# fenghuayumo/DIVSHOT

Hardware: AMD Instinct MI355X
Metric: train views/sec (fwd+bwd raster) at 1M splats 1920x1080 (higher is better)
Workload: dtype f32; 1 GPU; C3: 1000000 splats, 1920x1080, SH degree 3, 8 views per iteration sharded over 1 GPU(s) (BASELINE config C4), 8 view(s) per GPU per step as 1 multi-view pass(es) of 8 view(s) (dvs_raster_forward_views / dvs_raster_backward_*); absgrad=True, mode=batch, stagger=False, groups=1, views_per_group=8, early_gather=False, a9_chunks=1, async_forward=True, hip_graph=False, fwd_variant=quadrant, grad_mode=0, tile_bounds=canonical, shN_layout=tiled[N/64][45][64]

## Files before the change

### divshot_amd/_lib.py

```python
import ctypes as C
import os

_HERE = os.path.dirname(os.path.abspath(__file__))
LIB_PATH = os.environ.get("DVS_RASTER_LIB") or os.path.join(_HERE, "lib", "libdvsraster.so")


class DvsError(RuntimeError):
    pass


if not os.path.exists(LIB_PATH):
    raise ImportError(
        f"{LIB_PATH} is missing: build it with `make -C divshot_amd/csrc` (or __graft_entry__.build()). "
        "divshot_amd has no CPU fallback.")

lib = C.CDLL(LIB_PATH, mode=C.RTLD_GLOBAL)


class Splats(C.Structure):
    _fields_ = [("pos", C.c_void_p), ("sh0", C.c_void_p), ("shN", C.c_void_p), ("opacity", C.c_void_p),
                ("scale", C.c_void_p), ("rot", C.c_void_p), ("n", C.c_int32), ("_pad", C.c_int32)]


class Camera(C.Structure):
    _fields_ = [("view", C.c_float * 16), ("proj", C.c_float * 16), ("tan_fovx", C.c_float), ("tan_fovy", C.c_float),
                ("focal_x", C.c_float), ("focal_y", C.c_float), ("campos", C.c_float * 3), ("width", C.c_int32),
                ("height", C.c_int32), ("bg", C.c_float * 3)]


class Opts(C.Structure):
    _fields_ = [("sh_degree", C.c_int32), ("antialias", C.c_int32), ("absgrad", C.c_int32), ("accumulate", C.c_int32),
                ("shn_layout", C.c_int32), ("grad_mode", C.c_int32), ("tile_bounds", C.c_int32), ("_reserved", C.c_int32 * 1)]


class FwdState(C.Structure):
    _fields_ = [("radii", C.c_void_p), ("splat2d", C.c_void_p), ("depth", C.c_void_p), ("flags", C.c_void_p), ("tiles_touched", C.c_void_p), ("sorted_tile", C.c_void_p),
                ("sorted_splat", C.c_void_p), ("ranges", C.c_void_p), ("final_T", C.c_void_p), ("n_contrib", C.c_void_p),
                ("num_rendered", C.c_uint64), ("n", C.c_int32), ("width", C.c_int32), ("height", C.c_int32),
                ("tiles_x", C.c_int32), ("tiles_y", C.c_int32), ("_pad", C.c_int32)]


class SplatGrads(C.Structure):
    _fields_ = [("pos", C.c_void_p), ("sh0", C.c_void_p), ("shN", C.c_void_p), ("opacity", C.c_void_p),
                ("scale", C.c_void_p), ("rot", C.c_void_p), ("absgrad2d", C.c_void_p), ("mean2d", C.c_void_p), ("dcolor", C.c_void_p)]


class DensifyParams(C.Structure):
    _fields_ = [("grad_threshold", C.c_float), ("scale_threshold", C.c_float), ("min_opacity", C.c_float), ("max_world_scale", C.c_float),
                ("max_screen_radius", C.c_int32), ("cap_max", C.c_int32), ("seed", C.c_uint32), ("shn_layout", C.c_int32), ("revised_opacity", C.c_int32)]


class AdamGroup(C.Structure):
    _fields_ = [("param", C.c_void_p), ("grad", C.c_void_p), ("m", C.c_void_p), ("v", C.c_void_p), ("count", C.c_uint64),
                ("lr", C.c_float), ("width", C.c_int32), ("layout", C.c_int32), ("active_chunks", C.c_int32)]


class McmcSets(C.Structure):
    _fields_ = [("param", C.c_void_p * 6), ("m", C.c_void_p * 6), ("v", C.c_void_p * 6)]


class SceneSpec(C.Structure):
    _fields_ = [("n", C.c_int32), ("width", C.c_int32), ("height", C.c_int32), ("sh_degree", C.c_int32),
                ("n_cams", C.c_int32), ("seed", C.c_uint64), ("fov_x_deg", C.c_float), ("scale_log_offset", C.c_float)]


_PROTOS = {
    "dvs_create": (C.c_void_p, [C.c_int, C.c_size_t, C.c_int, C.c_int]),
    "dvs_create_views": (C.c_void_p, [C.c_int, C.c_size_t, C.c_int, C.c_int, C.c_int]),
    "dvs_destroy": (None, [C.c_void_p]),
    "dvs_raster_forward_views": (C.c_int, [C.c_void_p, C.c_void_p, C.POINTER(Splats), C.POINTER(Camera), C.c_int, C.POINTER(Opts), C.c_void_p]),
    "dvs_raster_forward_cancel_prepared": (C.c_int, [C.c_void_p]),
    "dvs_raster_forward_views_prepare": (C.c_int, [C.c_void_p, C.c_void_p, C.POINTER(Splats), C.POINTER(Camera), C.c_int, C.POINTER(Opts), C.c_int64, C.c_int64]),
    "dvs_raster_backward_views": (C.c_int, [C.c_void_p, C.c_void_p, C.POINTER(Splats), C.POINTER(Camera), C.c_int, C.POINTER(Opts),
                                            C.c_void_p, C.POINTER(SplatGrads)]),
    "dvs_get_view_state": (C.c_int, [C.c_void_p, C.c_int, C.POINTER(FwdState)]),
    "dvs_raster_forward": (C.c_int, [C.c_void_p, C.c_void_p, C.POINTER(Splats), C.POINTER(Camera), C.POINTER(Opts),
                                     C.c_void_p, C.POINTER(FwdState), C.POINTER(C.c_uint64)]),
    "dvs_raster_backward": (C.c_int, [C.c_void_p, C.c_void_p, C.POINTER(Splats), C.POINTER(Camera), C.POINTER(Opts),
                                      C.c_void_p, C.POINTER(SplatGrads)]),
    "dvs_raster_backward_composite": (C.c_int, [C.c_void_p, C.c_void_p, C.c_void_p, C.POINTER(Opts), C.c_void_p]),
    "dvs_raster_backward_project": (C.c_int, [C.c_void_p, C.c_void_p, C.POINTER(Splats), C.c_void_p, C.POINTER(Opts),
                                              C.POINTER(SplatGrads)]),
    "dvs_raster_backward_project_chunk": (C.c_int, [C.c_void_p, C.c_void_p, C.POINTER(Splats), C.c_void_p, C.POINTER(Opts),
                                                    C.POINTER(SplatGrads), C.c_int64, C.c_int64]),
    "dvs_raster_backward_dcolor": (C.c_int, [C.c_void_p, C.c_void_p, C.c_void_p]),
    "dvs_sh_grad_combine": (C.c_int, [C.c_void_p, C.c_void_p, C.c_int, C.c_void_p, C.c_int, C.c_int, C.c_void_p, C.c_void_p, C.c_void_p,
                                      C.c_void_p, C.c_int, C.c_int]),
    "dvs_shn_relayout": (C.c_int, [C.c_void_p, C.c_void_p, C.c_int, C.c_void_p, C.c_void_p, C.c_int]),
    "dvs_sort_pairs_u32": (C.c_int, [C.c_void_p, C.c_void_p, C.c_void_p, C.c_void_p, C.c_uint64, C.c_int, C.c_int]),
    "dvs_export_sorted_keys": (C.c_int, [C.c_void_p, C.c_void_p, C.c_void_p]),
    "dvs_get_bwd_intermediates": (C.c_int, [C.c_void_p, C.POINTER(C.c_void_p), C.POINTER(C.c_int)]),
    "dvs_keep_bwd_intermediates": (C.c_int, [C.c_void_p, C.c_int]),
    "dvs_set_async": (C.c_int, [C.c_void_p, C.c_int]),
    "dvs_get_num_rendered": (C.c_int, [C.c_void_p, C.c_void_p, C.POINTER(C.c_uint64)]),
    "dvs_get_sort_rank_mode": (C.c_int, [C.c_void_p]),
    "dvs_debug_sort_depth_keys": (C.c_int, [C.c_void_p, C.c_void_p, C.c_void_p, C.c_uint64, C.c_void_p, C.POINTER(C.c_uint32), C.POINTER(C.c_uint32)]),
    "dvs_set_export_sorted_tiles": (C.c_int, [C.c_void_p, C.c_int]),
    "dvs_get_arena_info": (C.c_int, [C.c_void_p, C.POINTER(C.c_uint64), C.POINTER(C.c_uint64), C.POINTER(C.c_uint64), C.POINTER(C.c_uint64)]),
    "dvs_set_backward_variant": (C.c_int, [C.c_void_p, C.c_int]),
    "dvs_debug_record_decisions": (C.c_int, [C.c_void_p, C.c_void_p, C.c_uint64]),
    "dvs_set_forward_variant": (C.c_int, [C.c_void_p, C.c_int]),
    "dvs_set_live_lists": (C.c_int, [C.c_void_p, C.c_int]),
    "dvs_enable_stage_timing": (C.c_int, [C.c_void_p, C.c_int]),
    "dvs_enable_kernel_probe": (C.c_int, [C.c_void_p, C.c_int]),
    "dvs_read_kernel_probe": (C.c_int, [C.c_void_p, C.POINTER(C.c_float), C.POINTER(C.c_int)]),
    "dvs_get_stage_timing": (C.c_int, [C.c_void_p, C.POINTER(C.POINTER(C.c_char_p)), C.POINTER(C.POINTER(C.c_float))]),
    "dvs_memcpy_d2h": (C.c_int, [C.c_void_p, C.c_void_p, C.c_void_p, C.c_size_t]),
    "dvs_memcpy_h2d": (C.c_int, [C.c_void_p, C.c_void_p, C.c_void_p, C.c_size_t]),
    "dvs_device_malloc": (C.c_void_p, [C.c_void_p, C.c_size_t]),
    "dvs_device_free": (None, [C.c_void_p, C.c_void_p]),
    "dvs_comm_create": (C.c_void_p, [C.c_int, C.c_int, C.c_int, C.c_char_p, C.c_int]),
    "dvs_comm_bootstrap": (C.c_int, [C.c_int, C.c_int, C.c_char_p, C.c_int, C.c_void_p]),
    "dvs_comm_destroy": (None, [C.c_void_p]),
    "dvs_comm_rank": (C.c_int, [C.c_void_p]),
    "dvs_comm_world": (C.c_int, [C.c_void_p]),
    "dvs_comm_backend_ranks": (C.c_int, [C.c_void_p]),
    "dvs_comm_backend_name": (C.c_char_p, [C.c_void_p]),
    "dvs_comm_all_reduce_sum_f32": (C.c_int, [C.c_void_p, C.c_void_p, C.c_void_p, C.c_size_t]),
    "dvs_comm_all_reduce_max_i32": (C.c_int, [C.c_void_p, C.c_void_p, C.c_void_p, C.c_size_t]),
    "dvs_comm_reduce_scatter_sum_f32": (C.c_int, [C.c_void_p, C.c_void_p, C.c_void_p, C.c_void_p, C.c_size_t]),
    "dvs_comm_all_gather_f32": (C.c_int, [C.c_void_p, C.c_void_p, C.c_void_p, C.c_void_p, C.c_size_t]),
    "dvs_comm_broadcast": (C.c_int, [C.c_void_p, C.c_void_p, C.c_void_p, C.c_size_t, C.c_int]),
    "dvs_comm_group_start": (C.c_int, [C.c_void_p]),
    "dvs_comm_group_end": (C.c_int, [C.c_void_p]),
    "dvs_last_error": (C.c_char_p, []),
    "dvs_version": (C.c_char_p, []),
    "dvs_synth_splats": (C.c_int, [C.POINTER(SceneSpec)] + [C.c_void_p] * 6),
    "dvs_synth_camera": (C.c_int, [C.POINTER(SceneSpec), C.c_int, C.POINTER(Camera)]),
    "dvs_synth_target": (C.c_int, [C.POINTER(SceneSpec), C.c_int, C.c_void_p]),
    "dvs_make_camera": (C.c_int, [C.c_void_p, C.c_void_p, C.c_float, C.c_int, C.c_int, C.POINTER(Camera)]),
    "dvs_l1_loss_grad": (C.c_int, [C.c_void_p, C.c_void_p, C.c_void_p, C.c_size_t, C.c_void_p, C.c_void_p]),
    "dvs_l1_loss_grad_w": (C.c_int, [C.c_void_p, C.c_void_p, C.c_void_p, C.c_size_t, C.c_float, C.c_void_p, C.c_void_p]),
    "dvs_l2_loss_grad": (C.c_int, [C.c_void_p, C.c_void_p, C.c_void_p, C.c_size_t, C.c_float, C.c_void_p, C.c_void_p]),
    "dvs_ssim_forward": (C.c_int, [C.c_void_p, C.c_void_p, C.c_void_p, C.c_int, C.c_int, C.c_void_p, C.c_void_p, C.c_void_p, C.c_void_p]),
    "dvs_ssim_backward": (C.c_int, [C.c_void_p, C.c_void_p, C.c_void_p, C.c_int, C.c_int, C.c_void_p, C.c_void_p, C.c_void_p, C.c_float,
                                    C.c_void_p, C.c_int]),
    "dvs_loss_l1_ssim_backward": (C.c_int, [C.c_void_p, C.c_void_p, C.c_void_p, C.c_int, C.c_int, C.c_void_p, C.c_void_p, C.c_void_p, C.c_float,
                                            C.c_void_p, C.c_void_p]),
    "dvs_densify_accumulate": (C.c_int, [C.c_void_p, C.c_int, C.c_void_p, C.c_void_p, C.c_int, C.c_int, C.c_void_p, C.c_void_p, C.c_void_p]),
    "dvs_densify_accumulate_rows": (C.c_int, [C.c_void_p, C.c_int, C.c_int, C.c_void_p, C.c_void_p, C.c_int, C.c_int, C.c_void_p, C.c_void_p, C.c_void_p]),
    "dvs_any_view_radius": (C.c_int, [C.c_void_p, C.c_int, C.c_int, C.c_void_p, C.c_void_p]),
    "dvs_densify_plan": (C.c_int, [C.c_void_p, C.c_int, C.c_void_p, C.c_void_p, C.c_void_p, C.c_void_p, C.c_void_p, C.POINTER(DensifyParams),
                                   C.c_void_p, C.c_void_p, C.c_void_p, C.c_void_p]),
    "dvs_densify_apply": (C.c_int, [C.c_void_p, C.c_int, C.c_void_p, C.c_void_p, C.POINTER(DensifyParams), C.c_int, C.c_void_p, C.c_void_p, C.c_int]),
    "dvs_reset_opacity": (C.c_int, [C.c_void_p, C.c_int, C.c_void_p, C.c_float, C.c_void_p, C.c_void_p]),
    "dvs_adam_step": (C.c_int, [C.c_void_p, C.c_void_p, C.c_void_p, C.c_void_p, C.c_void_p, C.c_size_t, C.c_float, C.c_float,
                                C.c_float, C.c_float, C.c_int]),
    "dvs_mcmc_scratch_bytes": (C.c_size_t, [C.c_int]),
    "dvs_mcmc_init_scratch": (C.c_int, [C.c_void_p, C.c_void_p, C.c_int]),
    "dvs_mcmc_relocate": (C.c_int, [C.c_void_p, C.c_int, C.POINTER(McmcSets), C.c_float, C.c_uint32, C.c_int, C.c_void_p, C.c_int, C.c_void_p]),
    "dvs_mcmc_grow": (C.c_int, [C.c_void_p, C.c_int, C.c_int, C.POINTER(McmcSets), C.c_float, C.c_uint32, C.c_int, C.c_void_p, C.c_int]),
    "dvs_mcmc_add_noise": (C.c_int, [C.c_void_p, C.c_int, C.c_void_p, C.c_void_p, C.c_void_p, C.c_void_p, C.c_float, C.c_uint32]),
    "dvs_mcmc_regularize": (C.c_int, [C.c_void_p, C.c_int, C.c_void_p, C.c_void_p, C.c_void_p, C.c_void_p, C.c_float, C.c_float]),
    "dvs_mcmc_add_noise_range": (C.c_int, [C.c_void_p, C.c_int, C.c_int, C.c_int, C.c_void_p, C.c_void_p, C.c_void_p, C.c_void_p, C.c_float, C.c_uint32]),
    "dvs_mcmc_regularize_range": (C.c_int, [C.c_void_p, C.c_int, C.c_int, C.c_int, C.c_void_p, C.c_void_p, C.c_void_p, C.c_void_p, C.c_float, C.c_float]),
    "dvs_adam_step_groups": (C.c_int, [C.c_void_p, C.POINTER(AdamGroup), C.c_int, C.c_float, C.c_float, C.c_float, C.c_int, C.c_void_p,
                                       C.c_int32]),
}
for _name, (_res, _args) in _PROTOS.items():
    _f = getattr(lib, _name)
    _f.restype = _res
    _f.argtypes = _args


def check(status, what="dvs call"):
    if status != 0:
        raise DvsError(f"{what} failed with status {status}: {lib.dvs_last_error().decode()}")
```

### divshot_amd/csrc/dvs_api.cpp

```cpp
#include <hip/hip_runtime.h>
#include <cstdio>
#include <cstdlib>
#include <cstdint>
#include <cstring>
#include <mutex>
#include <string>
#include <vector>
#include "../../include/dvs_raster.h"
#include "dvs_kernels.h"

static thread_local std::string g_last_error;
static void set_error(const char* what, hipError_t e, const char* file, int line) {
    char buf[512];
    snprintf(buf, sizeof buf, "%s: %s (%s:%d)", what, hipGetErrorString(e), file, line);
    g_last_error = buf;
}
void dvs_set_last_error(const char* msg) { g_last_error = msg ? msg : ""; }
#define HIPCHECK(expr)                                                   \
    do {                                                                 \
        hipError_t _e = (expr);                                          \
        if (_e != hipSuccess) { set_error(#expr, _e, __FILE__, __LINE__); return DVS_ERR_HIP; } \
    } while (0)

namespace {
struct Buf {
    void* p = nullptr;
    size_t bytes = 0;
    int ensure(size_t need) {
        if (need <= bytes) return DVS_OK;
        if (p) { (void)hipFree(p); p = nullptr; bytes = 0; }
        size_t want = need + need / 4;
        hipError_t e = hipMalloc(&p, want);
        if (e != hipSuccess) { e = hipMalloc(&p, need); want = need; }
        if (e != hipSuccess) { set_error("hipMalloc", e, __FILE__, __LINE__); p = nullptr; return DVS_ERR_HIP; }
        bytes = want;
#ifdef DVS_EXPERIMENT
        (void)hipMemset(p, 0, want);
#endif
        return DVS_OK;
    }
    void release() { if (p) (void)hipFree(p); p = nullptr; bytes = 0; }
    template <class T> T* as() const { return (T*)p; }
};

DvsCam to_dev_cam(const dvs_camera& c) {
    DvsCam d;
    memcpy(d.view, c.view, sizeof d.view); memcpy(d.proj, c.proj, sizeof d.proj);
    d.tan_fovx = c.tan_fovx; d.tan_fovy = c.tan_fovy; d.focal_x = c.focal_x; d.focal_y = c.focal_y;
    memcpy(d.campos, c.campos, sizeof d.campos);
    d.width = c.width; d.height = c.height; memcpy(d.bg, c.bg, sizeof d.bg);
    return d;
}
int bits_for(uint32_t max_value) { int b = 0; while (max_value) { ++b; max_value >>= 1; } return b; }
}

struct dvs_ctx {
    int device = 0;
    size_t max_splats = 0;
    int max_w = 0, max_h = 0;
    int max_views = 1;
    int n_views = 1;
    Buf radii, splat2d, depth, flags, tiles_touched, rect, rect_sorted, key[2], ids[2];
    Buf inst_tile[2], inst_splat[2];
    uint32_t* live_splat = nullptr;
    uint32_t* live_pos = nullptr;
    bool live_lists = true;
    Buf tmp_keys, tmp_vals;
    bool export_tiles = false;
    int fe_rank_atomic = 0;
    Buf ranges_canon;
    Buf ranges, final_T, n_contrib;
    size_t fe_zero_bytes = 0;
    uint32_t fe_nbv = 0, fe_nsb = 0;
    Buf fe_state;
    Buf fe_hist;
    int fe_seg_n = -1, fe_seg_V = -1;
    uint32_t fe_seg_rows = 0;
    Buf g_rows;
    Buf dcolor;
    uint64_t* total_dev = nullptr;
    uint64_t* total_host = nullptr;
    uint64_t inst_cap = 0;
    uint64_t inst_grow_events = 0;
    bool async_T = false;
    uint64_t* rec_masks = nullptr; uint64_t rec_cap = 0;
    uint64_t overflow_seen = 0;
    dvs_fwd_state st{};
    bool have_fwd = false;
    bool keep_rows = false;
    bool rows_clean = false;
    bool rows_pending = false;
    int64_t proj_next = 0;
    struct Prep {
        bool valid = false;
        int64_t next = 0;
        int n = 0, V = 0;
        dvs_splats p{};
        dvs_opts opts{};
        dvs_camera cams[DVS_MAX_VIEWS];
    } prep;
    int bwd_variant = DVS_BWD_TR;
    int fwd_variant = DVS_FWD_QUADRANT;
    bool timing = false;
    bool probe = false;
    std::vector<hipEvent_t> probe_ev;
    std::vector<int> probe_kind;
    size_t probe_used = 0;
    std::vector<hipEvent_t> events;
    std::vector<const char*> ev_names;
    size_t ev_used = 0;
    std::vector<const char*> out_names;
    std::vector<float> out_ms;
    std::vector<std::pair<const char*, std::pair<size_t, size_t>>> spans;
};

namespace {
struct StageTimer {
    dvs_ctx* c; hipStream_t st;
    StageTimer(dvs_ctx* c_, hipStream_t s) : c(c_), st(s) {}
    size_t mark() {
        if (!c->timing) return 0;
        if (c->ev_used == c->events.size()) { hipEvent_t e; (void)hipEventCreate(&e); c->events.push_back(e); }
        (void)hipEventRecord(c->events[c->ev_used], st);
        return c->ev_used++;
    }
    void span(const char* name, size_t a, size_t b) { if (c->timing) c->spans.push_back({name, {a, b}}); }
};
void timing_reset(dvs_ctx* c) { c->ev_used = 0; c->spans.clear(); }
hipEvent_t probe_event(dvs_ctx* c, hipStream_t st) {
    if (c->probe_used == c->probe_ev.size()) { hipEvent_t e; (void)hipEventCreate(&e); c->probe_ev.push_back(e); }
    hipEvent_t e = c->probe_ev[c->probe_used++];
    (void)hipEventRecord(e, st);
    return e;
}
void timing_collect(dvs_ctx* c, bool append) {
    if (!c->timing) return;
    if (!append) { c->out_names.clear(); c->out_ms.clear(); }
    for (auto& s : c->spans) {
        float ms = 0.f;
        (void)hipEventSynchronize(c->events[s.second.second]);
        (void)hipEventElapsedTime(&ms, c->events[s.second.first], c->events[s.second.second]);
        c->out_names.push_back(s.first); c->out_ms.push_back(ms);
    }
}

bool fe_no_key16() { static const bool v = [] { const char* e = getenv("DVS_FE_NO_KEY16"); return e && e[0] == '1'; }(); return v; }
bool fe_no_fuse() { static const bool v = [] { const char* e = getenv("DVS_FE_NO_FUSE_A6"); return e && e[0] == '1'; }(); return v; }
uint32_t* ranges_ptr(dvs_ctx* c) { return (uint32_t*)((char*)c->ranges.p + c->fe_zero_bytes); }
uint32_t* fe_kred(dvs_ctx* c) { return (uint32_t*)c->ranges.p; }
unsigned long long* fe_super(dvs_ctx* c) { return (unsigned long long*)((char*)c->ranges.p + (size_t)DVS_FE_KRED_WORDS * 4); }
DvsSeg* fe_seg_all(dvs_ctx* c) { return c->fe_state.as<DvsSeg>(); }
DvsSeg* fe_seg_vis(dvs_ctx* c) { return c->fe_state.as<DvsSeg>() + DVS_MAX_VIEWS; }
DvsSeg* fe_seg_tile(dvs_ctx* c) { return c->fe_state.as<DvsSeg>() + 2 * DVS_MAX_VIEWS; }
uint32_t* fe_superexcl(dvs_ctx* c) { return (uint32_t*)(c->fe_state.as<DvsSeg>() + 3 * DVS_MAX_VIEWS); }
uint32_t* fe_totals(dvs_ctx* c) { return fe_superexcl(c) + (size_t)c->max_views * c->fe_nsb; }
uint32_t* fe_block_sums(dvs_ctx* c) { return fe_totals(c) + (size_t)c->max_views * DVS_FE_MAXBINS; }
int ensure_frontend_arenas(dvs_ctx* c) {
    dvs_fe_block_counts((int)c->max_splats, &c->fe_nbv, &c->fe_nsb);
    c->fe_zero_bytes = (size_t)DVS_FE_KRED_WORDS * 4 + (size_t)c->max_views * c->fe_nsb * 8 * DVS_FE_SUPER_STRIDE;
    c->fe_zero_bytes = (c->fe_zero_bytes + 255) & ~(size_t)255;
    int r;
    const size_t state = 3 * DVS_MAX_VIEWS * sizeof(DvsSeg) + ((size_t)c->max_views * c->fe_nsb + (size_t)c->max_views * DVS_FE_MAXBINS + (size_t)c->max_views * c->fe_nbv) * 4;
    if ((r = c->fe_state.ensure(state)) != DVS_OK) return r;
    if ((r = c->fe_hist.ensure(dvs_fe_hist_words((uint64_t)c->max_splats * c->max_views, c->max_views, DVS_FE_MAXBINS) * 4)) != DVS_OK) return r;
    return DVS_OK;
}

int ensure_splat_arenas(dvs_ctx* c, size_t n) {
    int r;
#define ENS(buf, bytes) if ((r = c->buf.ensure(bytes)) != DVS_OK) return r;
    ENS(radii, n * 4) ENS(splat2d, n * 64) ENS(depth, n * 4)
    ENS(flags, n * 4) ENS(tiles_touched, n * 4) ENS(rect, n * 16) ENS(rect_sorted, n * 16)      ENS(key[0], n * 4) ENS(key[1], n * 4) ENS(ids[0], n * 4) ENS(ids[1], n * 4)
    ENS(g_rows, n * 48)
#undef ENS
    return DVS_OK;
}
int ensure_image_arenas(dvs_ctx* c, int w, int h, int views) {
    const size_t P = (size_t)w * h * views;
    const size_t tiles = (size_t)((w + DVS_TILE - 1) / DVS_TILE) * ((h + DVS_TILE - 1) / DVS_TILE) * views;
    int r;
    if ((r = c->ranges.ensure(c->fe_zero_bytes + tiles * 8)) != DVS_OK) return r;
    if ((r = c->ranges_canon.ensure(tiles * 8)) != DVS_OK) return r;
    if ((r = c->final_T.ensure(P * 4)) != DVS_OK) return r;
    if ((r = c->n_contrib.ensure(P * 4)) != DVS_OK) return r;
    return DVS_OK;
}
int ensure_instance_arenas(dvs_ctx* c, uint64_t T) {
    int r;
    if (c->inst_cap && T > c->inst_cap) ++c->inst_grow_events;
    for (int k = 0; k < 2; ++k) {
        if ((r = c->inst_tile[k].ensure(T * 4)) != DVS_OK) return r;
        if ((r = c->inst_splat[k].ensure(T * 4)) != DVS_OK) return r;
    }
    c->inst_cap = c->inst_tile[0].bytes / 4;
    for (int k = 0; k < 2; ++k) {
        if (c->inst_tile[k].bytes / 4 < c->inst_cap) c->inst_cap = c->inst_tile[k].bytes / 4;
        if (c->inst_splat[k].bytes / 4 < c->inst_cap) c->inst_cap = c->inst_splat[k].bytes / 4;
    }
    if (c->inst_cap >= (1ull << 32)) c->inst_cap = (1ull << 32) - 1;
    if ((r = c->fe_hist.ensure(dvs_fe_hist_words(c->inst_cap, c->max_views, 512) * 4)) != DVS_OK) return r;
    return DVS_OK;
}
}

extern "C" {

const char* dvs_last_error(void) { return g_last_error.c_str(); }
const char* dvs_version(void) { return "divshot_amd raster 0.1 (gfx950)"; }

dvs_ctx* dvs_create_views(int device, size_t max_splats, int max_w, int max_h, int max_views) {
    int count = 0;
    hipError_t e = hipGetDeviceCount(&count);
    if (e != hipSuccess || device < 0 || device >= count) {
        g_last_error = "dvs_create: no such HIP device (the rasterizer has no CPU fallback)";
        return nullptr;
    }
    if (max_views < 1 || max_views > DVS_MAX_VIEWS) { g_last_error = "dvs_create_views: max_views must be in [1, 16]"; return nullptr; }
    if ((e = hipSetDevice(device)) != hipSuccess) { set_error("hipSetDevice", e, __FILE__, __LINE__); return nullptr; }
    dvs_ctx* c = new dvs_ctx();
    c->device = device; c->max_splats = max_splats; c->max_w = max_w; c->max_h = max_h; c->max_views = max_views;
    if (const char* v = getenv("DVS_BWD_VARIANT")) {
        c->bwd_variant = v[0] == '0' ? DVS_BWD_BLOCKS : v[0] == '1' ? DVS_BWD_REDUCE : v[0] == '2' ? DVS_BWD_MM : DVS_BWD_TR;
        if ((c->bwd_variant == DVS_BWD_REDUCE || c->bwd_variant == DVS_BWD_MM) && !dvs_launch_render_bwd) c->bwd_variant = DVS_BWD_TR;
    }
    if (const char* v = getenv("DVS_FWD_VARIANT")) c->fwd_variant = (v[0] == '0' && dvs_launch_render_fwd_blocks) ? DVS_FWD_BLOCKS : DVS_FWD_QUADRANT;
    if (const char* v = getenv("DVS_LIVE_LISTS")) c->live_lists = v[0] != '0';
    if (hipMalloc((void**)&c->total_dev, 32) != hipSuccess || hipHostMalloc((void**)&c->total_host, 32, hipHostMallocDefault) != hipSuccess ||
        hipMemset(c->total_dev, 0, 32) != hipSuccess) {
        g_last_error = "dvs_create: hipMalloc failed";
        delete c;
        return nullptr;
    }
    c->total_host[0] = c->total_host[1] = c->total_host[2] = c->total_host[3] = 0;
    {
        static int probed[64];
        static std::mutex probe_mutex;
        std::lock_guard<std::mutex> probe_lock(probe_mutex);
        const char* mode = getenv("DVS_FE_RANK");
        if (mode && mode[0] == 'b') c->fe_rank_atomic = 0;
        else {
            if (device < 64 && probed[device] == 0) {
                uint32_t bad = 1u;
                uint32_t* word = nullptr;
                if (hipMalloc((void**)&word, 4) == hipSuccess && hipMemset(word, 0, 4) == hipSuccess && dvs_fe_probe_rank_atomic(nullptr, word) == hipSuccess &&
                    hipMemcpy(&bad, word, 4, hipMemcpyDeviceToHost) == hipSuccess)
                    probed[device] = bad == 0u ? 1 : 2;
                if (word) (void)hipFree(word);
            }
            c->fe_rank_atomic = (device < 64 && probed[device] == 1) ? 1 : 0;
        }
    }
    if (const char* v = getenv("DVS_ASYNC")) c->async_T = v[0] == '1';
    if (ensure_frontend_arenas(c) != DVS_OK ||
        ensure_splat_arenas(c, max_splats * (size_t)max_views) != DVS_OK || ensure_image_arenas(c, max_w, max_h, max_views) != DVS_OK ||
        ensure_instance_arenas(c, (uint64_t)max_splats * 4 * (uint64_t)max_views) != DVS_OK) {
        dvs_destroy(c);
        return nullptr;
    }
    return c;
}
dvs_ctx* dvs_create(int device, size_t max_splats, int max_w, int max_h) { return dvs_create_views(device, max_splats, max_w, max_h, 1); }

void dvs_destroy(dvs_ctx* c) {
    if (!c) return;
    (void)hipSetDevice(c->device);
    Buf* all[] = {&c->radii, &c->splat2d, &c->depth, &c->flags, &c->tiles_touched, &c->rect, &c->rect_sorted, &c->key[0], &c->key[1],
                  &c->ids[0], &c->ids[1], &c->inst_tile[0], &c->inst_tile[1], &c->inst_splat[0], &c->inst_splat[1],
                  &c->tmp_keys, &c->tmp_vals, &c->ranges, &c->final_T, &c->n_contrib, &c->g_rows, &c->dcolor, &c->fe_state, &c->fe_hist, &c->ranges_canon};
    for (Buf* b : all) b->release();
    if (c->total_dev) (void)hipFree(c->total_dev);
    if (c->total_host) (void)hipHostFree(c->total_host);
    for (hipEvent_t e : c->events) (void)hipEventDestroy(e);
    for (hipEvent_t e : c->probe_ev) (void)hipEventDestroy(e);
    delete c;
}

static int run_a2(dvs_ctx* c, hipStream_t st, const dvs_splats* p, const dvs_camera* cams, int V, const dvs_opts* opts, int64_t first, int64_t count, bool begin) {
    const int n = p->n, W = cams[0].width, H = cams[0].height;
    const int tiles_x = (W + DVS_TILE - 1) / DVS_TILE, tiles_y = (H + DVS_TILE - 1) / DVS_TILE, tiles = tiles_x * tiles_y;
    const int tight = opts->tile_bounds == DVS_TILES_TIGHT ? 1 : 0;
    const int rect_fmt = tight ? DVS_FE_RECT_TIGHT : (tiles_x <= 255 && tiles_y <= 255) ? DVS_FE_RECT_U8 : DVS_FE_RECT_U16;
    DvsCams dcams;
    for (int v = 0; v < V; ++v) dcams.c[v] = to_dev_cam(cams[v]);
    if (begin) HIPCHECK(hipMemsetAsync(c->ranges.p, 0, c->fe_zero_bytes + (size_t)tiles * V * 8, st));
    HIPCHECK(dvs_launch_preprocess_fwd(st, n, p->pos, p->sh0, p->shN, p->opacity, p->scale, p->rot, dcams, V, opts->sh_degree,
                                       opts->antialias, tiles_x, tiles_y, c->radii.as<int>(), c->splat2d.as<float>(),
                                       c->depth.as<float>(), c->flags.as<uint32_t>(), c->tiles_touched.as<uint32_t>(), c->key[0].as<uint32_t>(),
                                       nullptr, opts->shn_layout, rect_fmt == DVS_FE_RECT_U16 ? c->rect.as<uint32_t>() : nullptr,
                                       rect_fmt == DVS_FE_RECT_TIGHT ? c->rect.as<uint32_t>() : nullptr,
                                       rect_fmt == DVS_FE_RECT_U8 ? c->rect.as<uint32_t>() : nullptr, fe_kred(c), (int)first, (int)count));
    return DVS_OK;
}
static bool prep_matches(const dvs_ctx* c, const dvs_splats* p, const dvs_camera* cams, int V, const dvs_opts* opts) {
    const dvs_ctx::Prep& q = c->prep;
    return q.valid && q.n == p->n && q.V == V && memcmp(&q.p, p, sizeof *p) == 0 && memcmp(&q.opts, opts, sizeof *opts) == 0 &&
           memcmp(q.cams, cams, sizeof(dvs_camera) * (size_t)V) == 0;
}

static int forward_views(dvs_ctx* c, hipStream_t st, const dvs_splats* p, const dvs_camera* cams, int V, const dvs_opts* opts,
                         float* out_rgb, dvs_fwd_state* saved, uint64_t* num_rendered) {
    const dvs_camera* cam = &cams[0];
    const int n = p->n, W = cam->width, H = cam->height;
    const int tiles_x = (W + DVS_TILE - 1) / DVS_TILE, tiles_y = (H + DVS_TILE - 1) / DVS_TILE, tiles = tiles_x * tiles_y;
    const size_t nV = (size_t)n * V;
    DvsCams dcams;
    float bgs[DVS_MAX_VIEWS * 3];
    for (int v = 0; v < V; ++v) { dcams.c[v] = to_dev_cam(cams[v]); for (int k = 0; k < 3; ++k) bgs[3 * v + k] = cams[v].bg[k]; }
    c->have_fwd = false;
    c->rows_pending = false;
    timing_reset(c);
    StageTimer tm(c, st);
    const int tight = opts->tile_bounds == DVS_TILES_TIGHT ? 1 : 0;

    uint64_t T = 0, T_expected = 0;
    const uint64_t* T_dev = nullptr;
    int icur = 0;
    size_t e7 = 0;
    int ranges_encoded = 0;
    bool keys_written = true;
    if (c->async_T) {
        const uint64_t lastT = c->total_host[0], overflow = c->total_host[1];
        if (overflow != c->overflow_seen) {
            c->overflow_seen = overflow;
            HIPCHECK(hipStreamSynchronize(st));
            int r = ensure_instance_arenas(c, lastT + lastT / 2);
            if (r != DVS_OK) return r;
            g_last_error = "dvs_raster_forward (async): an earlier forward on this context produced more tile instances than the instance "
                           "arena held; its outputs are invalid. The arena has been enlarged — repeat that view.";
            return DVS_ERR_CAPACITY;
        }
        if (lastT + lastT / 8 > c->inst_cap) {
            HIPCHECK(hipStreamSynchronize(st));
            int r = ensure_instance_arenas(c, lastT + lastT / 2);
            if (r != DVS_OK) return r;
        }
        T = c->inst_cap;
        T_dev = c->total_dev;
        T_expected = lastT > 0 ? lastT + lastT / 16 + 4096 : 0;
    }
    {
        const int rect_fmt = tight ? DVS_FE_RECT_TIGHT : (tiles_x <= 255 && tiles_y <= 255) ? DVS_FE_RECT_U8 : DVS_FE_RECT_U16;
        const bool prepared = prep_matches(c, p, cams, V, opts) && c->prep.next == (int64_t)n;
        c->prep.valid = false;
        size_t e0 = tm.mark();
        if (!prepared) { int r = run_a2(c, st, p, cams, V, opts, 0, n, true); if (r != DVS_OK) return r; }
        size_t e1 = tm.mark(); tm.span("preprocess_fwd", e0, e1);
        if (n > 0) {
            const uint32_t rows = dvs_depth_sort_rows_per_view(n, V);
            if (c->fe_seg_n != n || c->fe_seg_V != V || c->fe_seg_rows != rows) {
                HIPCHECK(dvs_launch_seg_init(st, n, V, rows, fe_seg_all(c)));
                c->fe_seg_n = n; c->fe_seg_V = V; c->fe_seg_rows = rows;
            }
            HIPCHECK(dvs_launch_depth_sort(st, n, V, c->key[0].as<uint32_t>(), c->ids[0].as<uint32_t>(), c->key[1].as<uint32_t>(), c->ids[1].as<uint32_t>(),
                                           fe_seg_all(c), fe_seg_vis(c), fe_kred(c), c->fe_hist.as<uint32_t>(), fe_totals(c), c->fe_rank_atomic));
        }
        size_t e2 = tm.mark(); tm.span("depth_sort", e1, e2);
        const uint64_t lastT = c->total_host[0];
        const uint64_t t_hint = T_expected ? T_expected : (lastT ? lastT : (uint64_t)nV * 3);
        const uint32_t tile_part = dvs_fe_part_for(t_hint);
        if (n > 0)
            HIPCHECK(dvs_launch_seg_binning(st, n, V, rect_fmt, fe_seg_vis(c), fe_seg_tile(c), c->ids[1].as<uint32_t>(), c->rect.as<uint32_t>(),
                                            c->rect_sorted.as<uint32_t>(), fe_block_sums(c), fe_super(c), fe_superexcl(c), tile_part,
                                            (unsigned long long*)c->total_dev, c->async_T ? c->inst_cap : ~0ull, 0, tiles_x, nullptr, nullptr));
        else
            HIPCHECK(hipMemsetAsync(c->total_dev, 0, 8, st));
        HIPCHECK(hipMemcpyAsync(c->total_host, c->total_dev, 32, hipMemcpyDeviceToHost, st));
        size_t e3 = tm.mark(); tm.span("tile_scan", e2, e3);
        if (!c->async_T) {
            HIPCHECK(hipStreamSynchronize(st));
            T = c->total_host[0];
            if (T >= (1ull << 32)) { g_last_error = "dvs_raster_forward: more than 2^32 tile instances"; return DVS_ERR_CAPACITY; }
            { int r = ensure_instance_arenas(c, T ? T : 1); if (r != DVS_OK) return r; }
        }
        const int key16 = (tiles <= 65536 && !fe_no_key16()) ? 1 : 0;
        size_t e4 = tm.mark();
        if (n > 0)
            HIPCHECK(dvs_launch_seg_binning(st, n, V, rect_fmt, fe_seg_vis(c), fe_seg_tile(c), c->ids[1].as<uint32_t>(), c->rect.as<uint32_t>(),
                                            c->rect_sorted.as<uint32_t>(), fe_block_sums(c), fe_super(c), fe_superexcl(c), tile_part,
                                            (unsigned long long*)c->total_dev, c->inst_cap, 1, tiles_x, c->inst_tile[0].as<uint32_t>(),
                                            c->inst_splat[0].as<uint32_t>(), key16));
        size_t e5 = tm.mark(); tm.span("duplicate", e4, e5);
        const bool fuse_a6 = (c->fwd_variant == DVS_FWD_QUADRANT || V > 1) && !fe_no_fuse();
        const bool write_keys = !(fuse_a6 && c->async_T) || c->export_tiles;
        if (n > 0) {
            const uint64_t cap = c->async_T ? c->inst_cap : T;
            const uint32_t nbtot = (uint32_t)(cap / tile_part) + (uint32_t)V + 2u;
            HIPCHECK(dvs_launch_seg_sort(st, V, c->inst_tile[0].as<uint32_t>(), c->inst_splat[0].as<uint32_t>(), c->inst_tile[1].as<uint32_t>(),
                                         c->inst_splat[1].as<uint32_t>(), fe_seg_tile(c), 0, tiles > 1 ? bits_for((uint32_t)(tiles - 1)) : 1,
                                         c->async_T ? (T_expected ? T_expected : c->inst_cap) : T, tile_part, nbtot, c->fe_hist.as<uint32_t>(), fe_totals(c),
                                         (uint32_t)tiles, &icur, fuse_a6 ? ranges_ptr(c) : nullptr, write_keys ? 1 : 0, key16, c->fe_rank_atomic));
        }
        size_t e6 = tm.mark(); tm.span("tile_sort", e5, e6);
        if (fuse_a6) ranges_encoded = n > 0 ? 1 : 0;
        else HIPCHECK(dvs_launch_tile_ranges(st, T, c->inst_tile[icur].as<uint32_t>(), ranges_ptr(c), tiles * V, T_dev, T_expected, false));
        keys_written = write_keys;
        e7 = tm.mark(); tm.span("tile_ranges", e6, e7);
    }
    if (c->probe) { (void)probe_event(c, st); c->probe_kind.push_back(0); }
    c->live_splat = nullptr; c->live_pos = nullptr;
    uint64_t* rec_masks = nullptr; uint64_t rec_cap = 0;
    if (c->rec_masks && V == 1 && !c->async_T && (c->fwd_variant == DVS_FWD_QUADRANT)) {
        rec_masks = c->rec_masks; rec_cap = c->rec_cap;
        HIPCHECK(hipMemsetAsync(rec_masks, 0, (size_t)(T < rec_cap ? T : rec_cap) * 32, st));
    }
    if (c->fwd_variant == DVS_FWD_QUADRANT || V > 1) {
        if (c->live_lists && c->bwd_variant == DVS_BWD_TR) { c->live_splat = c->inst_splat[icur ^ 1].as<uint32_t>(); c->live_pos = c->inst_tile[icur ^ 1].as<uint32_t>(); }
        HIPCHECK(dvs_launch_render_fwd(st, W, H, tiles_x, tiles_y, V, ranges_ptr(c), c->inst_splat[icur].as<uint32_t>(),
                                       c->splat2d.as<float>(), bgs, out_rgb, c->final_T.as<float>(), c->n_contrib.as<uint32_t>(),
                                       c->live_splat, c->live_pos, rec_masks, rec_cap, ranges_encoded ? c->ranges_canon.as<uint32_t>() : nullptr));
    } else
        HIPCHECK(dvs_launch_render_fwd_blocks(st, W, H, tiles_x, tiles_y, ranges_ptr(c), c->inst_splat[icur].as<uint32_t>(),
                                              c->splat2d.as<float>(), cam->bg, out_rgb,
                                              c->final_T.as<float>(), c->n_contrib.as<uint32_t>()));
    if (c->probe) (void)probe_event(c, st);
    size_t e8 = tm.mark(); tm.span("render_fwd", e7, e8);

    dvs_fwd_state& s = c->st;
    s.radii = c->radii.as<int32_t>(); s.splat2d = c->splat2d.as<float>(); s.depth = c->depth.as<float>();
    s.flags = c->flags.as<uint32_t>();
    s.tiles_touched = c->tiles_touched.as<uint32_t>();
    s.sorted_tile = keys_written ? c->inst_tile[icur].as<uint32_t>() : nullptr; s.sorted_splat = c->inst_splat[icur].as<uint32_t>();
    s.ranges = ranges_encoded ? c->ranges_canon.as<uint32_t>() : ranges_ptr(c); s.final_T = c->final_T.as<float>(); s.n_contrib = c->n_contrib.as<uint32_t>();
    s.num_rendered = c->async_T ? DVS_T_UNKNOWN : T; s.n = n; s.width = W; s.height = H; s.tiles_x = tiles_x; s.tiles_y = tiles_y;
    s._pad = 0;
    c->n_views = V;
    c->have_fwd = true;
    if (saved) *saved = s;
    if (num_rendered) *num_rendered = c->async_T ? DVS_T_UNKNOWN : T;
    if (c->timing) { HIPCHECK(hipStreamSynchronize(st)); timing_collect(c, false); }
    return DVS_OK;
}

static int check_fwd_args(dvs_ctx* c, const dvs_splats* p, const dvs_camera* cams, int V, const dvs_opts* opts, const float* out_rgb) {
    if (!c || !p || !cams || !opts || !out_rgb) { g_last_error = "dvs_raster_forward: null argument"; return DVS_ERR_INVALID; }
    if (V < 1 || V > c->max_views) { g_last_error = "dvs_raster_forward: n_views exceeds the max_views given to dvs_create_views"; return DVS_ERR_CAPACITY; }
    const dvs_camera* cam = &cams[0];
    if (p->n < 0 || cam->width <= 0 || cam->height <= 0 || opts->sh_degree < 0 || opts->sh_degree > 3 ||
        (opts->shn_layout != DVS_SHN_ROWS && opts->shn_layout != DVS_SHN_TILED) ||
        (opts->tile_bounds != DVS_TILES_CANONICAL && opts->tile_bounds != DVS_TILES_TIGHT)) {
        g_last_error = "dvs_raster_forward: bad n / image size / sh_degree / shn_layout / tile_bounds"; return DVS_ERR_INVALID;
    }
    for (int v = 1; v < V; ++v)
        if (cams[v].width != cam->width || cams[v].height != cam->height) { g_last_error = "dvs_raster_forward: the views of a batch must share one image size"; return DVS_ERR_INVALID; }
    if (p->n > 0 && (((uintptr_t)p->pos | (uintptr_t)p->sh0 | (uintptr_t)p->shN | (uintptr_t)p->opacity | (uintptr_t)p->scale | (uintptr_t)p->rot) & 15u)) {
        g_last_error = "dvs_raster_forward: parameter arrays must be 16-byte aligned"; return DVS_ERR_INVALID;
    }
    if ((size_t)p->n > c->max_splats || cam->width > c->max_w || cam->height > c->max_h) {
        g_last_error = "dvs_raster_forward: exceeds the capacity given to dvs_create"; return DVS_ERR_CAPACITY;
    }
    if ((uint64_t)p->n * (uint64_t)V >= (1ull << 31)) { g_last_error = "dvs_raster_forward: n * n_views must stay below 2^31"; return DVS_ERR_CAPACITY; }
    return DVS_OK;
}

int dvs_raster_forward(dvs_ctx* c, void* stream, const dvs_splats* p, const dvs_camera* cam, const dvs_opts* opts,
                       float* out_rgb, dvs_fwd_state* saved, uint64_t* num_rendered) {
    int r = check_fwd_args(c, p, cam, 1, opts, out_rgb);
    if (r != DVS_OK) return r;
    HIPCHECK(hipSetDevice(c->device));
    return forward_views(c, (hipStream_t)stream, p, cam, 1, opts, out_rgb, saved, num_rendered);
}

int dvs_raster_forward_views(dvs_ctx* c, void* stream, const dvs_splats* p, const dvs_camera* cams, int n_views, const dvs_opts* opts,
                             float* out_rgb) {
    int r = check_fwd_args(c, p, cams, n_views, opts, out_rgb);
    if (r != DVS_OK) return r;
    HIPCHECK(hipSetDevice(c->device));
    return forward_views(c, (hipStream_t)stream, p, cams, n_views, opts, out_rgb, nullptr, nullptr);
}

int dvs_raster_forward_cancel_prepared(dvs_ctx* c) {
    if (!c) { g_last_error = "dvs_raster_forward_cancel_prepared: null context"; return DVS_ERR_INVALID; }
    c->prep.valid = false;
    return DVS_OK;
}
int dvs_raster_forward_views_prepare(dvs_ctx* c, void* stream, const dvs_splats* p, const dvs_camera* cams, int n_views, const dvs_opts* opts,
                                     int64_t first, int64_t count) {
    static float dummy_rgb;
    int r = check_fwd_args(c, p, cams, n_views, opts, &dummy_rgb);
    if (r != DVS_OK) return r;
    if (opts->shn_layout != DVS_SHN_TILED) { g_last_error = "dvs_raster_forward_views_prepare: needs the DVS_SHN_TILED layout"; return DVS_ERR_INVALID; }
    const bool begin = first == 0;
    if (!begin && !(prep_matches(c, p, cams, n_views, opts) && c->prep.next == first)) {
        c->prep.valid = false;
        g_last_error = "dvs_raster_forward_views_prepare: chunks must cover [0, n) in ascending order with the same parameters, cameras and options";
        return DVS_ERR_STATE;
    }
    if (count <= 0 || first < 0 || first + count > p->n || (first % 256) != 0) {
        c->prep.valid = false;
        g_last_error = "dvs_raster_forward_views_prepare: bad chunk (each starts at a multiple of 256 and lies inside [0, n))"; return DVS_ERR_INVALID;
    }
    HIPCHECK(hipSetDevice(c->device));
    if (begin) {
        c->have_fwd = false; c->rows_pending = false;
        c->prep.valid = true; c->prep.next = 0; c->prep.n = p->n; c->prep.V = n_views; c->prep.p = *p; c->prep.opts = *opts;
        memcpy(c->prep.cams, cams, sizeof(dvs_camera) * (size_t)n_views);
    }
    if ((r = run_a2(c, (hipStream_t)stream, p, cams, n_views, opts, first, count, begin)) != DVS_OK) { c->prep.valid = false; return r; }
    c->prep.next = first + count;
    return DVS_OK;
}

int dvs_get_view_state(dvs_ctx* c, int view, dvs_fwd_state* out) {
    if (!c || !out) { g_last_error = "dvs_get_view_state: null argument"; return DVS_ERR_INVALID; }
    if (!c->have_fwd || view < 0 || view >= c->n_views) { g_last_error = "dvs_get_view_state: no such view in the last forward"; return DVS_ERR_STATE; }
    dvs_fwd_state s = c->st;
    const size_t on = (size_t)view * s.n, op = (size_t)view * s.width * s.height, ot = (size_t)view * s.tiles_x * s.tiles_y;
    s.radii += on; s.splat2d += on * DVS_S2D_FLOATS; s.depth += on; s.flags += on; s.tiles_touched += on;
    s.ranges += 2 * ot; s.final_T += op; s.n_contrib += op;
    *out = s;
    return DVS_OK;
}

static int bwd_composite(dvs_ctx* c, hipStream_t st, const dvs_camera* cams, const dvs_opts* opts, const float* dL_drgb, StageTimer* tm) {
    const dvs_fwd_state& s = c->st;
    const int V = c->n_views;
    size_t e0 = tm ? tm->mark() : 0;
    if (!c->rows_clean) HIPCHECK(hipMemsetAsync(c->g_rows.p, 0, c->g_rows.bytes, st));
    c->rows_clean = false;
    size_t e1 = tm ? tm->mark() : 0;
    if (tm) tm->span("bwd_zero", e0, e1);
    float bgs[DVS_MAX_VIEWS * 3];
    for (int v = 0; v < V; ++v) for (int k = 0; k < 3; ++k) bgs[3 * v + k] = cams[v].bg[k];
    if (c->probe) { (void)probe_event(c, st); c->probe_kind.push_back(1); }
    if (c->bwd_variant == DVS_BWD_TR)
        HIPCHECK(dvs_launch_render_bwd_tr(st, s.width, s.height, s.tiles_x, s.tiles_y, V, s.ranges, s.sorted_splat, s.splat2d, bgs, s.final_T,
                                          s.n_contrib, dL_drgb, c->g_rows.as<float>(), opts->absgrad, opts->grad_mode, c->live_splat, c->live_pos));
    else if (c->bwd_variant == DVS_BWD_BLOCKS)
        HIPCHECK(dvs_launch_render_bwd_blocks(st, s.width, s.height, s.tiles_x, s.tiles_y, V, s.ranges, s.sorted_splat, s.splat2d,
                                              bgs, s.final_T, s.n_contrib, dL_drgb, c->g_rows.as<float>(), opts->absgrad, opts->grad_mode));
    else {
        if (!dvs_launch_render_bwd) { g_last_error = "dvs_raster_backward: this build does not contain the selected composite-backward variant"; return DVS_ERR_INVALID; }
        HIPCHECK(dvs_launch_render_bwd(st, s.width, s.height, s.tiles_x, s.tiles_y, V, s.ranges, s.sorted_splat, s.splat2d,
                                       bgs, s.final_T, s.n_contrib, dL_drgb, c->g_rows.as<float>(), opts->absgrad, opts->grad_mode,
                                       V > 1 ? DVS_BWD_REDUCE : c->bwd_variant));
    }
    if (c->probe) (void)probe_event(c, st);
    if (tm) { size_t e2 = tm->mark(); tm->span("render_bwd", e1, e2); }
    c->rows_pending = true;
    c->proj_next = 0;
    return DVS_OK;
}
static int bwd_project(dvs_ctx* c, hipStream_t st, const dvs_splats* p, const dvs_camera* cams, const dvs_opts* opts,
                       const dvs_splat_grads* out, StageTimer* tm) {
    const dvs_fwd_state& s = c->st;
    const int V = c->n_views, n = p->n;
    size_t e2 = tm ? tm->mark() : 0;
    if (opts->shn_layout == DVS_SHN_TILED) {
        DvsCams dcams;
        float campos[DVS_MAX_VIEWS * 3];
        for (int v = 0; v < V; ++v) { dcams.c[v] = to_dev_cam(cams[v]); for (int k = 0; k < 3; ++k) campos[3 * v + k] = cams[v].campos[k]; }
        const char* nf = getenv("DVS_A9_NO_FUSE_SH");
        const bool no_fuse = nf && nf[0] == '1';
        const bool fuse = !out->dcolor && out->sh0 && out->shN && !no_fuse;
        float* dcol = out->dcolor;
        if (!dcol && !fuse) { int r = c->dcolor.ensure((size_t)V * n * 3 * sizeof(float)); if (r != DVS_OK) return r; dcol = c->dcolor.as<float>(); }
        HIPCHECK(dvs_launch_preprocess_bwd_views(st, n, V, p->pos, p->shN, p->opacity, p->scale, p->rot, dcams, opts->sh_degree,
                                                 opts->antialias, s.radii, s.flags, c->g_rows.as<float>(), out->pos, out->opacity, out->scale,
                                                 out->rot, opts->absgrad ? out->absgrad2d : nullptr, out->mean2d, dcol, opts->accumulate,
                                                 c->keep_rows ? 0 : 1, opts->grad_mode, 0, -1, fuse ? out->sh0 : nullptr, fuse ? out->shN : nullptr));
        if (!fuse && out->sh0 && out->shN)
            HIPCHECK(dvs_launch_sh_grad_combine(st, n, p->pos, opts->sh_degree, V, campos, dcol, out->sh0, out->shN, opts->accumulate, 1));
    } else {
        for (int v = 0; v < V; ++v) {
            const DvsCam dcam = to_dev_cam(cams[v]);
            const size_t on = (size_t)v * n;
            HIPCHECK(dvs_launch_preprocess_bwd(st, n, p->pos, p->shN, p->opacity, p->scale, p->rot, dcam, opts->sh_degree, opts->antialias,
                                               s.radii + on, s.flags + on, c->g_rows.as<float>() + on * 12, out->pos, out->sh0, out->shN,
                                               out->opacity, out->scale, out->rot, opts->absgrad ? out->absgrad2d : nullptr, out->mean2d,
                                               out->dcolor ? out->dcolor + on * 3 : nullptr, (opts->accumulate || v > 0) ? 1 : 0,
                                               c->keep_rows ? 0 : 1, opts->shn_layout, opts->grad_mode));
        }
    }
    c->rows_clean = !c->keep_rows;
    c->rows_pending = c->keep_rows;
    c->proj_next = 0;
    if (tm) { size_t e3 = tm->mark(); tm->span("preprocess_bwd", e2, e3); }
    return DVS_OK;
}
static int check_bwd_args(dvs_ctx* c, const dvs_splats* p, const dvs_camera* cams, int V, const dvs_opts* opts, const char* who) {
    static thread_local std::string msg;
    if (!c || !cams || !opts) { msg = std::string(who) + ": null argument"; g_last_error = msg.c_str(); return DVS_ERR_INVALID; }
    if (opts->grad_mode != DVS_GRAD_TRUE && opts->grad_mode != DVS_GRAD_LINEAGE) { msg = std::string(who) + ": bad grad_mode"; g_last_error = msg.c_str(); return DVS_ERR_INVALID; }
    if (!c->have_fwd || V != c->n_views || (p && c->st.n != p->n) || c->st.width != cams[0].width || c->st.height != cams[0].height) {
        msg = std::string(who) + ": no matching forward on this context"; g_last_error = msg.c_str(); return DVS_ERR_STATE;
    }
    return DVS_OK;
}
static int check_grads(const dvs_splats* p, const dvs_splat_grads* out, const char* who) {
    static thread_local std::string msg;
    if (!p || !out) { msg = std::string(who) + ": null argument"; g_last_error = msg.c_str(); return DVS_ERR_INVALID; }
    if (p->n > 0 && (!out->pos || !out->opacity || !out->scale || !out->rot || ((!out->sh0 || !out->shN) && !out->dcolor))) {
        msg = std::string(who) + ": null gradient row pointer (sh0/shN may be NULL only when dcolor is given)";
        g_last_error = msg.c_str(); return DVS_ERR_INVALID;
    }
    if (p->n > 0 && (((uintptr_t)out->pos | (uintptr_t)out->sh0 | (uintptr_t)out->shN | (uintptr_t)out->opacity | (uintptr_t)out->scale |
                      (uintptr_t)out->rot | (uintptr_t)out->absgrad2d | (uintptr_t)out->mean2d | (uintptr_t)out->dcolor) & 15u)) {
        msg = std::string(who) + ": gradient arrays must be 16-byte aligned"; g_last_error = msg.c_str(); return DVS_ERR_INVALID;
    }
    return DVS_OK;
}

static int backward_views(dvs_ctx* c, void* stream, const dvs_splats* p, const dvs_camera* cams, int V, const dvs_opts* opts,
                          const float* dL_drgb, const dvs_splat_grads* out, const char* who) {
    int r;
    if (!dL_drgb) { g_last_error = "dvs_raster_backward: null argument"; return DVS_ERR_INVALID; }
    if ((uintptr_t)dL_drgb & 15u) { g_last_error = "dvs_raster_backward: dL_drgb must be 16-byte aligned (the composite backward reads it as 16-byte words)"; return DVS_ERR_INVALID; }
    if ((r = check_grads(p, out, who)) != DVS_OK) return r;
    if ((r = check_bwd_args(c, p, cams, V, opts, who)) != DVS_OK) return r;
    HIPCHECK(hipSetDevice(c->device));
    hipStream_t st = (hipStream_t)stream;
    timing_reset(c);
    StageTimer tm(c, st);
    if ((r = bwd_composite(c, st, cams, opts, dL_drgb, &tm)) != DVS_OK) return r;
    if ((r = bwd_project(c, st, p, cams, opts, out, &tm)) != DVS_OK) return r;
    if (c->timing) { HIPCHECK(hipStreamSynchronize(st)); timing_collect(c, true); }
    return DVS_OK;
}
int dvs_raster_backward(dvs_ctx* c, void* stream, const dvs_splats* p, const dvs_camera* cam, const dvs_opts* opts,
                        const float* dL_drgb, const dvs_splat_grads* out) {
    return backward_views(c, stream, p, cam, 1, opts, dL_drgb, out, "dvs_raster_backward");
}
int dvs_raster_backward_views(dvs_ctx* c, void* stream, const dvs_splats* p, const dvs_camera* cams, int n_views, const dvs_opts* opts,
                              const float* dL_drgb, const dvs_splat_grads* out) {
    return backward_views(c, stream, p, cams, n_views, opts, dL_drgb, out, "dvs_raster_backward_views");
}

int dvs_raster_backward_composite(dvs_ctx* c, void* stream, const dvs_camera* cam, const dvs_opts* opts, const float* dL_drgb) {
    int r;
    if (!dL_drgb) { g_last_error = "dvs_raster_backward_composite: null argument"; return DVS_ERR_INVALID; }
    if ((uintptr_t)dL_drgb & 15u) { g_last_error = "dvs_raster_backward_composite: dL_drgb must be 16-byte aligned (the composite backward reads it as 16-byte words)"; return DVS_ERR_INVALID; }
    if (!c) { g_last_error = "dvs_raster_backward_composite: null argument"; return DVS_ERR_INVALID; }
    if ((r = check_bwd_args(c, nullptr, cam, c->n_views, opts, "dvs_raster_backward_composite")) != DVS_OK) return r;
    HIPCHECK(hipSetDevice(c->device));
    timing_reset(c);
    StageTimer tm(c, (hipStream_t)stream);
    if ((r = bwd_composite(c, (hipStream_t)stream, cam, opts, dL_drgb, &tm)) != DVS_OK) return r;
    if (c->timing) { HIPCHECK(hipStreamSynchronize((hipStream_t)stream)); timing_collect(c, true); }
    return DVS_OK;
}

int dvs_raster_backward_project(dvs_ctx* c, void* stream, const dvs_splats* p, const dvs_camera* cam, const dvs_opts* opts,
                                const dvs_splat_grads* out) {
    int r;
    if ((r = check_grads(p, out, "dvs_raster_backward_project")) != DVS_OK) return r;
    if (!c) { g_last_error = "dvs_raster_backward_project: null argument"; return DVS_ERR_INVALID; }
    if ((r = check_bwd_args(c, p, cam, c->n_views, opts, "dvs_raster_backward_project")) != DVS_OK) return r;
    if (!c->rows_pending) { g_last_error = "dvs_raster_backward_project: no dvs_raster_backward_composite on this context"; return DVS_ERR_STATE; }
    if (c->proj_next != 0) {
        g_last_error = "dvs_raster_backward_project: a dvs_raster_backward_project_chunk sequence is in progress on this context (finish it up to n)";
        return DVS_ERR_STATE;
    }
    HIPCHECK(hipSetDevice(c->device));
    timing_reset(c);
    StageTimer tm(c, (hipStream_t)stream);
    if ((r = bwd_project(c, (hipStream_t)stream, p, cam, opts, out, &tm)) != DVS_OK) return r;
    if (c->timing) { HIPCHECK(hipStreamSynchronize((hipStream_t)stream)); timing_collect(c, true); }
    return DVS_OK;
}

int dvs_raster_backward_project_chunk(dvs_ctx* c, void* stream, const dvs_splats* p, const dvs_camera* cam, const dvs_opts* opts,
                                      const dvs_splat_grads* out, int64_t first, int64_t count) {
    int r;
    if ((r = check_grads(p, out, "dvs_raster_backward_project_chunk")) != DVS_OK) return r;
    if (!c) { g_last_error = "dvs_raster_backward_project_chunk: null argument"; return DVS_ERR_INVALID; }
    if ((r = check_bwd_args(c, p, cam, c->n_views, opts, "dvs_raster_backward_project_chunk")) != DVS_OK) return r;
    if (!c->rows_pending) { g_last_error = "dvs_raster_backward_project_chunk: no dvs_raster_backward_composite pending on this context"; return DVS_ERR_STATE; }
    if (opts->shn_layout != DVS_SHN_TILED || !out->dcolor || out->sh0 || out->shN) {
        g_last_error = "dvs_raster_backward_project_chunk: needs the DVS_SHN_TILED layout and the factorised form (out->dcolor given, sh0 / shN NULL)";
        return DVS_ERR_INVALID;
    }
    if (first != c->proj_next || count <= 0 || first + count > p->n || (first % 256) != 0) {
        g_last_error = "dvs_raster_backward_project_chunk: chunks must cover [0, n) in ascending order, each starting at a multiple of 256";
        return DVS_ERR_INVALID;
    }
    HIPCHECK(hipSetDevice(c->device));
    const dvs_fwd_state& s = c->st;
    const int V = c->n_views, n = p->n;
    DvsCams dcams;
    for (int v = 0; v < V; ++v) dcams.c[v] = to_dev_cam(cam[v]);
    timing_reset(c);
    StageTimer tm(c, (hipStream_t)stream);
    const size_t t0 = tm.mark();
    HIPCHECK(dvs_launch_preprocess_bwd_views((hipStream_t)stream, n, V, p->pos, p->shN, p->opacity, p->scale, p->rot, dcams, opts->sh_degree,
                                             opts->antialias, s.radii, s.flags, c->g_rows.as<float>(), out->pos, out->opacity, out->scale,
                                             out->rot, opts->absgrad ? out->absgrad2d : nullptr, out->mean2d, out->dcolor, opts->accumulate,
                                             c->keep_rows ? 0 : 1, opts->grad_mode, (int)first, (int)count));
    { const size_t t1 = tm.mark(); tm.span("preprocess_bwd", t0, t1); }
    if (c->timing) { HIPCHECK(hipStreamSynchronize((hipStream_t)stream)); timing_collect(c, true); }
    c->proj_next = first + count;
    if (c->proj_next == n) { c->rows_clean = !c->keep_rows; c->rows_pending = c->keep_rows; c->proj_next = 0; }
    return DVS_OK;
}

int dvs_sort_pairs_u32(dvs_ctx* c, void* stream, uint32_t* keys, uint32_t* vals, uint64_t n, int bit_lo, int bit_hi) {
    if (!c || (n > 0 && (!keys || !vals)) || bit_lo < 0 || bit_hi > 32 || bit_lo > bit_hi) { g_last_error = "dvs_sort_pairs_u32: bad argument"; return DVS_ERR_INVALID; }
    HIPCHECK(hipSetDevice(c->device));
    hipStream_t st = (hipStream_t)stream;
    if (n == 0) return DVS_OK;
    int r;
    if ((r = c->tmp_keys.ensure(n * 4)) != DVS_OK) return r;
    if ((r = c->tmp_vals.ensure(n * 4)) != DVS_OK) return r;
    uint32_t* k[2] = {keys, c->tmp_keys.as<uint32_t>()};
    uint32_t* v[2] = {vals, c->tmp_vals.as<uint32_t>()};
    int cur = 0;
    {
        if (n > (1ull << 32) - 4097ull) { g_last_error = "dvs_sort_pairs_u32: n must be at most 2^32 - 4097"; return DVS_ERR_CAPACITY; }
        if ((r = c->fe_hist.ensure(dvs_fe_hist_words(n, 1, 512) * 4)) != DVS_OK) return r;
        const uint32_t part = dvs_fe_part_for(n);
        HIPCHECK(dvs_launch_seg_init(st, (int)n, 1, 0, fe_seg_all(c)));
        c->fe_seg_n = -1;
        HIPCHECK(dvs_launch_seg_sort(st, 1, k[0], v[0], k[1], v[1], fe_seg_all(c), bit_lo, bit_hi - bit_lo, n, part, (uint32_t)(n / part) + 3u,
                                     c->fe_hist.as<uint32_t>(), fe_totals(c), 0u, &cur, nullptr, 1, 0, c->fe_rank_atomic));
    }
    if (cur == 1) {
        HIPCHECK(hipMemcpyAsync(keys, k[1], n * 4, hipMemcpyDeviceToDevice, st));
        HIPCHECK(hipMemcpyAsync(vals, v[1], n * 4, hipMemcpyDeviceToDevice, st));
    }
    return DVS_OK;
}

int dvs_debug_sort_depth_keys(dvs_ctx* c, void* stream, const uint32_t* keys, uint64_t n, uint32_t* sorted_ids, uint32_t* n_sorted, uint32_t* digit_bits) {
    if (!c || !keys || !sorted_ids || !n_sorted || n == 0 || n > c->max_splats * (uint64_t)c->max_views || n >= (1ull << 31)) {
        g_last_error = "dvs_debug_sort_depth_keys: bad argument (n must be in [1, max_splats * max_views])"; return DVS_ERR_INVALID;
    }
    HIPCHECK(hipSetDevice(c->device));
    hipStream_t st = (hipStream_t)stream;
    std::vector<uint32_t> h(n);
    HIPCHECK(hipMemcpyAsync(h.data(), keys, n * 4, hipMemcpyDeviceToHost, st));
    HIPCHECK(hipStreamSynchronize(st));
    uint32_t mn = 0xFFFFFFFFu, mx = 0u; bool any = false;
    for (uint32_t k : h) if (k != 0xFFFFFFFFu) { mn = k < mn ? k : mn; mx = k > mx ? k : mx; any = true; }
    uint32_t slots[64 * 16] = {0};
    if (any) { slots[0] = ~mn; slots[1] = mx; }
    HIPCHECK(hipMemcpyAsync(fe_kred(c), slots, sizeof slots, hipMemcpyHostToDevice, st));
    HIPCHECK(hipMemcpyAsync(c->key[0].p, keys, n * 4, hipMemcpyDeviceToDevice, st));
    const uint32_t rows = dvs_depth_sort_rows_per_view((int)n, 1);
    HIPCHECK(dvs_launch_seg_init(st, (int)n, 1, rows, fe_seg_all(c)));
    c->fe_seg_n = -1;
    HIPCHECK(dvs_launch_depth_sort(st, (int)n, 1, c->key[0].as<uint32_t>(), c->ids[0].as<uint32_t>(), c->key[1].as<uint32_t>(), c->ids[1].as<uint32_t>(),
                                   fe_seg_all(c), fe_seg_vis(c), fe_kred(c), c->fe_hist.as<uint32_t>(), fe_totals(c), c->fe_rank_atomic));
    DvsSeg sv;
    HIPCHECK(hipMemcpyAsync(&sv, fe_seg_vis(c), sizeof sv, hipMemcpyDeviceToHost, st));
    HIPCHECK(hipStreamSynchronize(st));
    *n_sorted = sv.count;
    if (digit_bits) *digit_bits = sv.bits;
    HIPCHECK(hipMemcpyAsync(sorted_ids, c->ids[1].p, (size_t)sv.count * 4, hipMemcpyDeviceToDevice, st));
    HIPCHECK(hipMemsetAsync(fe_kred(c), 0, sizeof slots, st));
    c->have_fwd = false;
    return DVS_OK;
}

int dvs_export_sorted_keys(dvs_ctx* c, void* stream, uint64_t* out_keys) {
    if (!c || !out_keys) { g_last_error = "dvs_export_sorted_keys: null argument"; return DVS_ERR_INVALID; }
    if (!c->have_fwd) { g_last_error = "dvs_export_sorted_keys: no forward state"; return DVS_ERR_STATE; }
    if (c->st.num_rendered == DVS_T_UNKNOWN) { uint64_t t; int r = dvs_get_num_rendered(c, stream, &t); if (r != DVS_OK) return r; }
    if (!c->st.sorted_tile) {
        g_last_error = "dvs_export_sorted_keys: the last forward was asynchronous (dvs_set_async) and did not materialise the sorted tile ids; "
                       "export the keys of a synchronous forward";
        return DVS_ERR_STATE;
    }
    HIPCHECK(hipSetDevice(c->device));
    HIPCHECK(dvs_launch_export_keys((hipStream_t)stream, c->st.num_rendered, c->st.sorted_tile, c->st.sorted_splat, c->st.depth, out_keys));
    return DVS_OK;
}

int dvs_shn_relayout(dvs_ctx* c, void* stream, int n, const float* src, float* dst, int to_tiled) {
    if (!c || n < 0 || (n > 0 && (!src || !dst))) { g_last_error = "dvs_shn_relayout: bad argument"; return DVS_ERR_INVALID; }
    HIPCHECK(hipSetDevice(c->device));
    HIPCHECK(dvs_launch_shn_relayout((hipStream_t)stream, n, src, dst, to_tiled));
    return DVS_OK;
}

int dvs_sh_grad_combine(dvs_ctx* c, void* stream, int n, const float* pos, int sh_degree, int n_views, const float* campos,
                        const float* dcolor, float* g_sh0, float* g_shN, int accumulate, int shn_layout) {
    if (!c || n < 0 || n_views < 0 || sh_degree < 0 || sh_degree > 3 || (n > 0 && n_views > 0 && (!pos || !campos || !dcolor || !g_sh0 || !g_shN))) {
        g_last_error = "dvs_sh_grad_combine: bad argument"; return DVS_ERR_INVALID;
    }
    HIPCHECK(hipSetDevice(c->device));
    HIPCHECK(dvs_launch_sh_grad_combine((hipStream_t)stream, n, pos, sh_degree, n_views, campos, dcolor, g_sh0, g_shN, accumulate, shn_layout));
    return DVS_OK;
}

int dvs_raster_backward_dcolor(dvs_ctx* c, void* stream, float* dcolor) {
    if (!c || !dcolor || ((uintptr_t)dcolor & 15u)) { g_last_error = "dvs_raster_backward_dcolor: bad argument (dcolor: 16-byte aligned device array)"; return DVS_ERR_INVALID; }
    if (!c->rows_pending) { g_last_error = "dvs_raster_backward_dcolor: no dvs_raster_backward_composite pending on this context"; return DVS_ERR_STATE; }
    HIPCHECK(hipSetDevice(c->device));
    const dvs_fwd_state& s = c->st;
    HIPCHECK(dvs_launch_dcolor_from_rows((hipStream_t)stream, (int64_t)c->n_views * s.n, s.radii, s.flags, c->g_rows.as<float>(), dcolor));
    return DVS_OK;
}

int dvs_set_async(dvs_ctx* c, int enable) {
    if (!c) { g_last_error = "dvs_set_async: null context"; return DVS_ERR_INVALID; }
    c->async_T = enable != 0;
    return DVS_OK;
}
int dvs_get_num_rendered(dvs_ctx* c, void* stream, uint64_t* T) {
    if (!c || !T) { g_last_error = "dvs_get_num_rendered: null argument"; return DVS_ERR_INVALID; }
    if (!c->have_fwd) { g_last_error = "dvs_get_num_rendered: no forward state"; return DVS_ERR_STATE; }
    HIPCHECK(hipSetDevice(c->device));
    HIPCHECK(hipStreamSynchronize((hipStream_t)stream));
    *T = c->total_host[0];
    c->st.num_rendered = *T;
    if (c->total_host[1] != c->overflow_seen) {
        c->overflow_seen = c->total_host[1];
        (void)ensure_instance_arenas(c, *T + *T / 2);
        g_last_error = "dvs_get_num_rendered: the last forward produced more tile instances than the instance arena held; its outputs are "
                       "invalid. The arena has been enlarged — repeat that view.";
        return DVS_ERR_CAPACITY;
    }
    return DVS_OK;
}

int dvs_get_sort_rank_mode(dvs_ctx* c) { return c ? c->fe_rank_atomic : -1; }
int dvs_set_export_sorted_tiles(dvs_ctx* c, int enable) {
    if (!c) { g_last_error = "dvs_set_export_sorted_tiles: null context"; return DVS_ERR_INVALID; }
    c->export_tiles = enable != 0;
    return DVS_OK;
}

int dvs_get_arena_info(dvs_ctx* c, uint64_t* cap, uint64_t* grows, uint64_t* last_T, uint64_t* overflows) {
    if (!c) { g_last_error = "dvs_get_arena_info: null context"; return DVS_ERR_INVALID; }
    if (cap) *cap = c->inst_cap;
    if (grows) *grows = c->inst_grow_events;
    if (last_T) *last_T = c->total_host[0];
    if (overflows) *overflows = c->total_host[1];
    return DVS_OK;
}

int dvs_debug_record_decisions(dvs_ctx* c, uint64_t* take_masks, uint64_t capacity_instances) {
    if (!c || (take_masks && (((uintptr_t)take_masks & 7u) || capacity_instances == 0))) { g_last_error = "dvs_debug_record_decisions: bad argument"; return DVS_ERR_INVALID; }
    c->rec_masks = take_masks; c->rec_cap = take_masks ? capacity_instances : 0;
    return DVS_OK;
}

int dvs_set_backward_variant(dvs_ctx* c, int variant) {
    if (!c || variant < DVS_BWD_BLOCKS || variant > DVS_BWD_TR) { g_last_error = "dvs_set_backward_variant: bad argument"; return DVS_ERR_INVALID; }
    if ((variant == DVS_BWD_REDUCE || variant == DVS_BWD_MM) && !dvs_launch_render_bwd) {
        g_last_error = "dvs_set_backward_variant: the 'reduce' and 'mm' kernels are retired — this library contains 'tr' (default) and 'blocks' only "
                       "(an experiment build, tools/xbuild.sh, brings them back)";
        return DVS_ERR_UNSUPPORTED;
    }
    c->bwd_variant = variant;
    return DVS_OK;
}
int dvs_set_live_lists(dvs_ctx* c, int enable) {
    if (!c) { g_last_error = "dvs_set_live_lists: null context"; return DVS_ERR_INVALID; }
    c->live_lists = enable != 0;
    return DVS_OK;
}
int dvs_set_forward_variant(dvs_ctx* c, int variant) {
    if (!c || (variant != DVS_FWD_BLOCKS && variant != DVS_FWD_QUADRANT)) { g_last_error = "dvs_set_forward_variant: bad argument"; return DVS_ERR_INVALID; }
    if (variant == DVS_FWD_BLOCKS && !dvs_launch_render_fwd_blocks) {
        g_last_error = "dvs_set_forward_variant: the per-block forward is retired — this library contains the quadrant forward only (tools/xbuild.sh brings it back)";
        return DVS_ERR_UNSUPPORTED;
    }
    c->fwd_variant = variant;
    return DVS_OK;
}

int dvs_keep_bwd_intermediates(dvs_ctx* c, int keep) { if (!c) return DVS_ERR_INVALID; c->keep_rows = keep != 0; return DVS_OK; }

int dvs_get_bwd_intermediates(dvs_ctx* c, const float** rows, int* row_floats) {
    if (!c) return DVS_ERR_INVALID;
    if (rows) *rows = c->g_rows.as<float>();
    if (row_floats) *row_floats = 12;
    return DVS_OK;
}

int dvs_enable_stage_timing(dvs_ctx* c, int enable) { if (!c) return DVS_ERR_INVALID; c->timing = enable != 0; return DVS_OK; }
int dvs_enable_kernel_probe(dvs_ctx* c, int enable) {
    if (!c) return DVS_ERR_INVALID;
    c->probe = enable != 0;
    c->probe_used = 0; c->probe_kind.clear();
    return DVS_OK;
}
int dvs_read_kernel_probe(dvs_ctx* c, float mean_ms[2], int count[2]) {
    if (!c || !mean_ms || !count) return DVS_ERR_INVALID;
    HIPCHECK(hipSetDevice(c->device));
    double sum[2] = {0, 0};
    count[0] = count[1] = 0;
    for (size_t k = 0; k < c->probe_kind.size() && 2 * k + 1 < c->probe_used; ++k) {
        float ms = 0.f;
        HIPCHECK(hipEventSynchronize(c->probe_ev[2 * k + 1]));
        HIPCHECK(hipEventElapsedTime(&ms, c->probe_ev[2 * k], c->probe_ev[2 * k + 1]));
        sum[c->probe_kind[k]] += ms; count[c->probe_kind[k]]++;
    }
    for (int i = 0; i < 2; ++i) mean_ms[i] = count[i] ? (float)(sum[i] / count[i]) : 0.f;
    c->probe_used = 0; c->probe_kind.clear();
    return DVS_OK;
}
int dvs_get_stage_timing(dvs_ctx* c, const char*** names, const float** ms) {
    if (!c) return 0;
    if (names) *names = c->out_names.data();
    if (ms) *ms = c->out_ms.data();
    return (int)c->out_names.size();
}

int dvs_memcpy_d2h(dvs_ctx* c, void* host_dst, const void* dev_src, size_t bytes) {
    if (!c) return DVS_ERR_INVALID;
    HIPCHECK(hipSetDevice(c->device));
    HIPCHECK(hipDeviceSynchronize());
    HIPCHECK(hipMemcpy(host_dst, dev_src, bytes, hipMemcpyDeviceToHost));
    return DVS_OK;
}
int dvs_memcpy_h2d(dvs_ctx* c, void* dev_dst, const void* host_src, size_t bytes) {
    if (!c) return DVS_ERR_INVALID;
    HIPCHECK(hipSetDevice(c->device));
    HIPCHECK(hipMemcpy(dev_dst, host_src, bytes, hipMemcpyHostToDevice));
    return DVS_OK;
}
void* dvs_device_malloc(dvs_ctx* c, size_t bytes) {
    if (!c) return nullptr;
    void* p = nullptr;
    if (hipSetDevice(c->device) != hipSuccess || hipMalloc(&p, bytes ? bytes : 1) != hipSuccess) return nullptr;
    return p;
}
void dvs_device_free(dvs_ctx* c, void* p) { if (c && p) { (void)hipSetDevice(c->device); (void)hipFree(p); } }

}
```

### divshot_amd/csrc/dvs_kernels.h

```cpp
#pragma once
#include <hip/hip_runtime.h>
#include <stdint.h>
#include "dvs_device.h"

hipError_t dvs_launch_preprocess_fwd(hipStream_t st, int n, const float* pos, const float* sh0, const float* shN,
                                     const float* opacity, const float* scale, const float* rot, const DvsCams& cams, int n_views,
                                     int deg, int antialias, int tiles_x, int tiles_y, int* radii , float* splat2d,
                                     float* depth, uint32_t* flags,
                                     uint32_t* tiles_touched, uint32_t* depth_key, uint32_t* ids, int shn_tiled, uint32_t* rect ,
                                     uint32_t* rect16 ,
                                     uint32_t* rect8 = nullptr ,
                                     uint32_t* kred = nullptr ,
                                     int first = 0, int count = -1 );
hipError_t dvs_launch_preprocess_bwd(hipStream_t st, int n, const float* pos, const float* shN, const float* opacity,
                                     const float* scale, const float* rot, const DvsCam& cam, int deg, int antialias,
                                     const int* radii, const uint32_t* flags, float* grad_rows ,
                                     float* g_pos, float* g_sh0, float* g_shN, float* g_opacity, float* g_scale,
                                     float* g_rot, float* out_absgrad2d , float* out_mean2d ,
                                     float* out_dcolor , int accumulate, int rezero_rows, int shn_tiled, int grad_mode);
hipError_t dvs_launch_preprocess_bwd_views(hipStream_t st, int n, int n_views, const float* pos, const float* shN, const float* opacity,
                                           const float* scale, const float* rot, const DvsCams& cams, int deg, int antialias,
                                           const int* radii, const uint32_t* flags, float* grad_rows, float* g_pos, float* g_opacity,
                                           float* g_scale, float* g_rot, float* out_absgrad2d, float* out_mean2d, float* out_dcolor,
                                           int accumulate, int rezero_rows, int grad_mode, int first = 0, int count = -1 ,
                                           float* g_sh0 = nullptr, float* g_shN = nullptr );
hipError_t dvs_launch_sh_grad_combine(hipStream_t st, int n, const float* pos, int deg, int n_views, const float* campos_host,
                                      const float* dcolor, float* g_sh0, float* g_shN, int accumulate, int shn_tiled);
hipError_t dvs_launch_dcolor_from_rows(hipStream_t st, int64_t total, const int* radii, const uint32_t* flags, const float* rows, float* dcolor);
hipError_t dvs_launch_shn_relayout(hipStream_t st, int n, const float* src, float* dst, int to_tiled);

struct DvsSeg {
    uint32_t base;
    uint32_t count;
    uint32_t pstart;
    uint32_t sub;
    uint32_t bits;
    uint32_t _r0, _r1, _r2;
};
enum { DVS_FE_RECT_U8 = 0 , DVS_FE_RECT_U16 = 1 ,
       DVS_FE_RECT_TIGHT = 2  };
#define DVS_FE_KRED_WORDS (DVS_MAX_VIEWS * 64 * 16)
#define DVS_FE_MAXBINS 2048
#define DVS_FE_SUPER_STRIDE 32
size_t dvs_fe_hist_words(uint64_t max_elems, int n_views, int max_bins);
uint32_t dvs_depth_sort_rows_per_view(int n, int V);
uint32_t dvs_fe_part_for(uint64_t grid_elems);
void dvs_fe_block_counts(int n, uint32_t* nbv, uint32_t* nsb);
hipError_t dvs_launch_seg_init(hipStream_t st, int n, int V, uint32_t rows_per_view, DvsSeg* seg_all);
hipError_t dvs_launch_depth_sort(hipStream_t st, int n, int V, uint32_t* keys0, uint32_t* vals0, uint32_t* keys1, uint32_t* vals1,
                                 DvsSeg* seg_all, DvsSeg* seg_vis, const uint32_t* kred, uint32_t* hist, uint32_t* totals ,
                                 int rank_atomic = 0 );
hipError_t dvs_launch_seg_sort(hipStream_t st, int V, uint32_t* keys0, uint32_t* vals0, uint32_t* keys1, uint32_t* vals1, DvsSeg* seg, int bit_lo, int bits,
                               uint64_t grid_elems, uint32_t part, uint32_t nbtot, uint32_t* hist, uint32_t* totals, uint32_t key_add_per_view,
                               int* result_in, uint32_t* ranges_enc = nullptr ,
                               int write_last_keys = 1, int first_keys16 = 0 , int rank_atomic = 0);
hipError_t dvs_fe_probe_rank_atomic(hipStream_t st, uint32_t* bad_dev);
hipError_t dvs_launch_seg_binning(hipStream_t st, int n, int V, int rect_fmt, const DvsSeg* seg_vis, DvsSeg* seg_tile, const uint32_t* sorted_ids,
                                  const uint32_t* rect, uint32_t* rect_sorted, uint32_t* block_sums, unsigned long long* super, uint32_t* superexcl,
                                  uint32_t tile_part, unsigned long long* total_dev, unsigned long long capacity, int stage, int tiles_x,
                                  uint32_t* inst_tile, uint32_t* inst_splat, int key16 = 0 );

hipError_t dvs_launch_tile_ranges(hipStream_t st, uint64_t T, const uint32_t* sorted_tile, uint32_t* ranges, int tiles,
                                  const uint64_t* T_dev = nullptr, uint64_t T_expected = 0, bool clear = true );
hipError_t dvs_launch_export_keys(hipStream_t st, uint64_t T, const uint32_t* sorted_tile, const uint32_t* sorted_splat,
                                  const float* depth, uint64_t* out_keys);

hipError_t dvs_launch_render_fwd(hipStream_t st, int W, int H, int tiles_x, int tiles_y, int n_views, const uint32_t* ranges ,
                                 const uint32_t* sorted_splat, const float* splat2d, const float* bgs, float* out_color, float* final_T,
                                 uint32_t* n_contrib, uint32_t* live_splat , uint32_t* live_pos ,
                                 uint64_t* take_masks ,
                                 uint64_t take_cap, uint32_t* ranges_out = nullptr );
hipError_t dvs_launch_render_bwd(hipStream_t st, int W, int H, int tiles_x, int tiles_y, int n_views, const uint32_t* ranges,
                                 const uint32_t* sorted_splat, const float* splat2d, const float* bgs, const float* final_T, const uint32_t* n_contrib,
                                 const float* dL_dout, float* grad_rows , int absgrad, int grad_mode,
                                 int variant ) __attribute__((weak));
enum { DVS_BWD_BLOCKS = 0 , DVS_BWD_REDUCE = 1 , DVS_BWD_MM = 2 ,
       DVS_BWD_TR = 3  };
enum { DVS_FWD_BLOCKS = 0 , DVS_FWD_QUADRANT = 1  };

hipError_t dvs_launch_render_bwd_tr(hipStream_t st, int W, int H, int tiles_x, int tiles_y, int n_views, const uint32_t* ranges,
                                    const uint32_t* sorted_splat, const float* splat2d, const float* bgs , const float* final_T,
                                    const uint32_t* n_contrib, const float* dL_dout, float* grad_rows, int absgrad, int grad_mode,
                                    const uint32_t* live_splat ,
                                    const uint32_t* live_pos);

hipError_t dvs_launch_render_fwd_blocks(hipStream_t st, int W, int H, int tiles_x, int tiles_y, const uint32_t* ranges,
                                        const uint32_t* sorted_splat, const float* splat2d, const float bg[3], float* out_color,
                                        float* final_T, uint32_t* n_contrib) __attribute__((weak));
hipError_t dvs_launch_render_bwd_blocks(hipStream_t st, int W, int H, int tiles_x, int tiles_y, int n_views, const uint32_t* ranges,
                                        const uint32_t* sorted_splat, const float* splat2d, const float* bgs , const float* final_T,
                                        const uint32_t* n_contrib, const float* dL_dout, float* grad_rows, int absgrad, int grad_mode);
```

### divshot_amd/csrc/frontend.hip

```cpp
#include <cstdlib>
#include "dvs_device.h"
#include "dvs_kernels.h"

#define FE_BLOCK 256
#define FE_WAVES (FE_BLOCK / 64)
#define FE_MAXBINS 2048
#define FE_REORDER_BITS 9
#define FE_CULLED 0xFFFFFFFFu

__device__ __forceinline__ uint32_t fe_lane() { return __builtin_amdgcn_mbcnt_hi(~0u, __builtin_amdgcn_mbcnt_lo(~0u, 0u)); }

__device__ __forceinline__ uint64_t fe_match(uint32_t d, bool valid, uint32_t b) {
    const uint64_t v0 = __ballot(valid);
    uint32_t lo = (uint32_t)v0, hi = (uint32_t)(v0 >> 32);
    for (uint32_t k = 0; k < b; ++k) {
        const uint32_t m = (uint32_t)(((int32_t)(d << (31u - k))) >> 31);
        const uint64_t bal = __ballot(m != 0u);
        lo = lo & ~((uint32_t)bal ^ m);
        hi = hi & ~((uint32_t)(bal >> 32) ^ m);
    }
    const uint64_t peers = ((uint64_t)hi << 32) | lo;
    return valid ? peers : 0ull;
}

__device__ __forceinline__ uint32_t fe_wave_incl_scan(uint32_t v) {
#define FE_DPP_ADD(ctrl, rmask) v += (uint32_t)__builtin_amdgcn_update_dpp(0, (int)v, ctrl, rmask, 0xF, false)
    FE_DPP_ADD(0x111, 0xF); FE_DPP_ADD(0x112, 0xF); FE_DPP_ADD(0x114, 0xF); FE_DPP_ADD(0x118, 0xF);
    FE_DPP_ADD(0x142, 0xA);
    FE_DPP_ADD(0x143, 0xC);
#undef FE_DPP_ADD
    return v;
}
__device__ __forceinline__ uint32_t fe_wave_sum(uint32_t v) { return (uint32_t)__builtin_amdgcn_readlane((int)fe_wave_incl_scan(v), 63); }

__device__ __forceinline__ uint32_t fe_block_excl_scan(uint32_t v, uint32_t* tmp, uint32_t* total) {
    const uint32_t lane = fe_lane(), wave = threadIdx.x >> 6;
    const uint32_t inc = fe_wave_incl_scan(v);
    if (lane == 63) tmp[wave] = inc;
    __syncthreads();
    uint32_t wbase = 0, tot = 0;
#pragma unroll
    for (int w = 0; w < FE_WAVES; ++w) { const uint32_t t = tmp[w]; if ((uint32_t)w < wave) wbase += t; tot += t; }
    __syncthreads();
    *total = tot;
    return wbase + inc - v;
}


template <int ITEMS>
__global__ void __launch_bounds__(FE_BLOCK)
k_seg_hist(const uint32_t* __restrict__ keys, DvsSeg* __restrict__ seg, int V, int adaptive, int pass, int shift_s, int bits_s, int cull,
           uint32_t* __restrict__ hist, uint32_t nbtot, const uint32_t* __restrict__ kred, int key16 ) {
    __shared__ uint32_t h[FE_MAXBINS];
    constexpr uint32_t PART = FE_BLOCK * ITEMS;
    const uint32_t lane = fe_lane(), wave = threadIdx.x >> 6, tid = threadIdx.x;
    const uint32_t view = blockIdx.x % (uint32_t)V, w = blockIdx.x / (uint32_t)V, gv = gridDim.x / (uint32_t)V;
    const uint32_t s_base = seg[view].base, s_count = seg[view].count, s_pstart = seg[view].pstart;
    uint32_t b = (uint32_t)bits_s, shift = (uint32_t)shift_s, sub = 0u;
    if (adaptive) {
        if (pass == 0) {
            uint32_t mn = ~kred[((size_t)view * 64 + lane) * 16], mx = kred[((size_t)view * 64 + lane) * 16 + 1];
#pragma unroll
            for (int d = 32; d >= 1; d >>= 1) {
                const uint32_t omn = __shfl_xor(mn, d, 64), omx = __shfl_xor(mx, d, 64);
                mn = omn < mn ? omn : mn; mx = omx > mx ? omx : mx;
            }
            sub = mn; b = 1u;
            if (mx >= mn) { const uint32_t range = mx - mn; const uint32_t rb = range ? 32u - (uint32_t)__builtin_clz(range) : 0u; b = (rb + 2u) / 3u; if (b < 1u) b = 1u; }
            else sub = 0u;
            if (w == 0 && tid == 0) { seg[view].sub = sub; seg[view].bits = b; }
        } else { sub = seg[view].sub; b = seg[view].bits; }
        shift = (uint32_t)pass * b;
    }
    const uint32_t nbins = 1u << b, dmask = nbins - 1u;
    const uint32_t nparts = (s_count + PART - 1) / PART;
    for (uint32_t p = w; p < nparts; p += gv) {
        for (uint32_t e = tid; e < nbins; e += FE_BLOCK) h[e] = 0u;
        __syncthreads();
        const uint32_t wb = p * PART + wave * (64 * ITEMS);
        uint32_t kreg[ITEMS];
        const uint32_t* const kin = keys + s_base;
        const uint16_t* const kin16 = reinterpret_cast<const uint16_t*>(keys) + s_base;
        const uint32_t i0 = wb + lane, ilast = s_count - 1u;
        if (key16) {
#pragma unroll
            for (int r = 0; r < ITEMS; ++r) { const uint32_t idx = i0 + (uint32_t)r * 64; kreg[r] = kin16[idx < ilast ? idx : ilast]; }
        } else {
#pragma unroll
            for (int r = 0; r < ITEMS; ++r) { const uint32_t idx = i0 + (uint32_t)r * 64; kreg[r] = kin[idx < ilast ? idx : ilast]; }
        }
#pragma unroll
        for (int r = 0; r < ITEMS; ++r) {
            const bool valid = i0 + (uint32_t)r * 64 <= ilast && !(cull && kreg[r] == FE_CULLED);
            if (valid) atomicAdd(&h[((kreg[r] - sub) >> shift) & dmask], 1u);
        }
        __syncthreads();
        const size_t row = (size_t)s_pstart + p;
        for (uint32_t d = tid; d < nbins; d += FE_BLOCK) hist[(size_t)d * nbtot + row] = h[d];
        __syncthreads();
    }
}

__global__ void __launch_bounds__(FE_BLOCK)
k_seg_rowscan(uint32_t* __restrict__ hist, uint32_t nbtot, const DvsSeg* __restrict__ seg, int V, int adaptive, int bits_s, uint32_t part,
              uint32_t* __restrict__ totals) {
    const uint32_t lane = fe_lane(), wave = threadIdx.x >> 6;
    const uint32_t view = blockIdx.x % (uint32_t)V, d = (blockIdx.x / (uint32_t)V) * FE_WAVES + wave;
    const uint32_t b = adaptive ? seg[view].bits : (uint32_t)bits_s;
    if (d >= (1u << b)) return;
    const uint32_t nparts = (seg[view].count + part - 1) / part;
    uint32_t* row = hist + (size_t)d * nbtot + seg[view].pstart;
    uint32_t carry = 0;
    for (uint32_t c0 = 0; c0 < nparts; c0 += 1024) {
        uint32_t v[16];
#pragma unroll
        for (int k = 0; k < 16; ++k) { const uint32_t i = c0 + (uint32_t)k * 64 + lane; v[k] = i < nparts ? row[i] : 0u; }
#pragma unroll
        for (int k = 0; k < 16; ++k) {
            if (c0 + (uint32_t)k * 64 < nparts) {
                const uint32_t i = c0 + (uint32_t)k * 64 + lane;
                const uint32_t inc = fe_wave_incl_scan(v[k]);
                if (i < nparts) row[i] = carry + inc - v[k];
                carry += (uint32_t)__builtin_amdgcn_readlane((int)inc, 63);
            }
        }
    }
    if (lane == 0) totals[(size_t)view * FE_MAXBINS + d] = carry;
}

template <int ITEMS> struct FeScatterLds {
    static constexpr int PART = FE_BLOCK * ITEMS;
    static constexpr int REORDER_WORDS = 1024 + 512 + 2 * PART;
    static constexpr int WIDE_WORDS = 4096 + 2048 + 2048;
    static constexpr int WORDS = (REORDER_WORDS > WIDE_WORDS ? REORDER_WORDS : WIDE_WORDS) + 8;
};

template <int ITEMS, bool RANK_ATOMIC >
__global__ void __launch_bounds__(FE_BLOCK) __attribute__((amdgpu_waves_per_eu(4)))
k_seg_scatter(const uint32_t* __restrict__ keys_in, const uint32_t* __restrict__ vals_in ,
              uint32_t* __restrict__ keys_out , uint32_t* __restrict__ vals_out,
              const DvsSeg* __restrict__ seg_in, DvsSeg* __restrict__ seg_out ,
              int V, int adaptive, int pass, int shift_s, int bits_s, int cull, uint32_t key_add_per_view,
              const uint32_t* __restrict__ hist, uint32_t nbtot, const uint32_t* __restrict__ totals,
              int key16 ,
              uint32_t* __restrict__ ranges_enc ) {
    constexpr uint32_t PART = FE_BLOCK * ITEMS;
    __shared__ __attribute__((aligned(16))) uint32_t lds[FeScatterLds<ITEMS>::WORDS];
    const uint32_t lane = fe_lane(), wave = threadIdx.x >> 6, tid = threadIdx.x;
    const uint32_t view = blockIdx.x % (uint32_t)V, w = blockIdx.x / (uint32_t)V, gv = gridDim.x / (uint32_t)V;
    const DvsSeg S = seg_in[view];
    const uint32_t b = adaptive ? S.bits : (uint32_t)bits_s;
    const uint32_t shift = adaptive ? (uint32_t)pass * b : (uint32_t)shift_s;
    const uint32_t sub = adaptive ? S.sub : 0u;
    const uint32_t nbins = 1u << b, dmask = nbins - 1u;
    const bool wide = b > FE_REORDER_BITS;
    const uint32_t cstride = wide ? 2048u : 512u;
    uint16_t* const cnt16 = reinterpret_cast<uint16_t*>(lds);
    uint32_t* const gdelta = lds + (wide ? 4096 : 1024);
    uint32_t* const dexl = lds + 6144;
    uint32_t* const stage_k = lds + 1536;
    uint32_t* const stage_v = stage_k + PART;
    uint32_t* const tmp = lds + (FeScatterLds<ITEMS>::WORDS - 8);
    const uint32_t key_add = key_add_per_view * view;
    const uint32_t* const vtot = totals + (size_t)view * FE_MAXBINS;
    const uint32_t* const kin = keys_in + S.base;
    const uint16_t* const kin16 = reinterpret_cast<const uint16_t*>(keys_in) + S.base;
    const uint32_t* const vin = vals_in ? vals_in + S.base : nullptr;
    uint32_t* const kout = keys_out ? keys_out + S.base : nullptr;
    uint32_t* const vout = vals_out + S.base;

    const uint32_t nparts = (S.count + PART - 1) / PART;
    const uint32_t ilast = S.count - 1u;
    uint32_t key[ITEMS], val[ITEMS], rank[ITEMS];
    constexpr bool EARLY = ITEMS <= 8;
    auto request = [&](uint32_t p) {
        const uint32_t i0 = p * PART + wave * (64 * ITEMS) + lane;
        if (key16) {
#pragma unroll
            for (int r = 0; r < ITEMS; ++r) { const uint32_t idx = i0 + (uint32_t)r * 64; key[r] = kin16[idx < ilast ? idx : ilast]; }
        } else {
#pragma unroll
            for (int r = 0; r < ITEMS; ++r) { const uint32_t idx = i0 + (uint32_t)r * 64; key[r] = kin[idx < ilast ? idx : ilast]; }
        }
        if (vin) {
#pragma unroll
            for (int r = 0; r < ITEMS; ++r) { const uint32_t idx = i0 + (uint32_t)r * 64; val[r] = vin[idx < ilast ? idx : ilast]; }
        } else {
#pragma unroll
            for (int r = 0; r < ITEMS; ++r) val[r] = i0 + (uint32_t)r * 64;
        }
    };
    if (EARLY && w < nparts) request(w);

    uint32_t dex0 = 0, dex1 = 0;
    {
        uint32_t s = 0;
        if (!wide) {
            const uint32_t t0 = 2u * tid < nbins ? vtot[2u * tid] : 0u, t1 = 2u * tid + 1u < nbins ? vtot[2u * tid + 1u] : 0u;
            dex1 = t0; s = t0 + t1;
        } else {
#pragma unroll 1
            for (uint32_t k = 0; k < 8; ++k) { const uint32_t d = tid * 8u + k; s += d < nbins ? vtot[d] : 0u; }
        }
        uint32_t tot;
        const uint32_t off = fe_block_excl_scan(s, tmp, &tot);
        if (!wide) { dex0 = off; dex1 += off; }
        else {
            uint32_t run = off;
#pragma unroll 1
            for (uint32_t k = 0; k < 8; ++k) { const uint32_t d = tid * 8u + k; dexl[d] = run; run += d < nbins ? vtot[d] : 0u; }
        }
        if (seg_out && w == 0 && tid == 0) { seg_out[view].base = S.base; seg_out[view].count = tot; seg_out[view].pstart = S.pstart; seg_out[view].sub = S.sub; seg_out[view].bits = S.bits; }
    }
    for (uint32_t p = w; p < nparts; p += gv) {
        const size_t row = (size_t)S.pstart + p;
        __syncthreads();
        for (uint32_t e = tid; e < cstride * 2u; e += FE_BLOCK) lds[e] = 0u;
        uint32_t hp0 = 0, hp1 = 0;
        if (!wide) {
            if (2u * tid < nbins) hp0 = hist[(size_t)(2u * tid) * nbtot + row];
            if (2u * tid + 1u < nbins) hp1 = hist[(size_t)(2u * tid + 1u) * nbtot + row];
        }
        if (!EARLY) request(p);
        __syncthreads();
        const uint32_t i0 = p * PART + wave * (64 * ITEMS) + lane;
        uint32_t vmask = 0u;
#pragma unroll
        for (int r = 0; r < ITEMS; ++r) {
            const bool valid = i0 + (uint32_t)r * 64 <= ilast && !(cull && key[r] == FE_CULLED);
            const uint32_t d = ((key[r] - sub) >> shift) & dmask;
            uint32_t prev = 0;
            if constexpr (RANK_ATOMIC) {
                if (valid) {
                    const uint32_t old = atomicAdd(&lds[wave * (cstride >> 1) + (d >> 1)], (d & 1u) ? 0x10000u : 1u);
                    prev = (d & 1u) ? (old >> 16) : (old & 0xFFFFu);
                    vmask |= 1u << r;
                }
                rank[r] = prev;
            } else {
                const uint64_t peers = fe_match(d, valid, b);
                const uint32_t below = __builtin_amdgcn_mbcnt_hi((uint32_t)(peers >> 32), __builtin_amdgcn_mbcnt_lo((uint32_t)peers, 0u));
                if (valid) {
                    prev = cnt16[wave * cstride + d];
                    if (below == 0) cnt16[wave * cstride + d] = (uint16_t)(prev + (uint32_t)__popcll(peers));
                    vmask |= 1u << r;
                }
                rank[r] = prev + below;
            }
            asm volatile("" : "+v"(rank[r]));
        }
        __syncthreads();
        if (!wide) {
            uint32_t c0[FE_WAVES], c1[FE_WAVES], bc0 = 0, bc1 = 0;
#pragma unroll
            for (int wv = 0; wv < FE_WAVES; ++wv) {
                const uint32_t two = *reinterpret_cast<const uint32_t*>(&cnt16[(uint32_t)wv * 512u + tid * 2u]);
                c0[wv] = two & 0xFFFFu; c1[wv] = two >> 16; bc0 += c0[wv]; bc1 += c1[wv];
            }
            uint32_t nvalid;
            uint32_t run = fe_block_excl_scan(bc0 + bc1, tmp, &nvalid);
            gdelta[tid * 2u] = dex0 + hp0 - run;
            gdelta[tid * 2u + 1u] = dex1 + hp1 - (run + bc0);
            uint32_t run1 = run + bc0;
#pragma unroll
            for (int wv = 0; wv < FE_WAVES; ++wv) {
                *reinterpret_cast<uint32_t*>(&cnt16[(uint32_t)wv * 512u + tid * 2u]) = run | (run1 << 16);
                run += c0[wv]; run1 += c1[wv];
            }
            __syncthreads();
#pragma unroll
            for (int r = 0; r < ITEMS; ++r) {
                if (vmask & (1u << r)) {
                    uint32_t kk = key[r];
                    asm volatile("" : "+v"(kk));
                    const uint32_t pos = cnt16[wave * 512u + (((kk - sub) >> shift) & dmask)] + rank[r];
                    stage_k[pos] = key[r];
                    stage_v[pos] = val[r];
                }
            }
            __syncthreads();
#pragma unroll
            for (int i = 0; i < ITEMS; ++i) {
                const uint32_t slot = (uint32_t)i * FE_BLOCK + tid;
                if (slot < nvalid) {
                    const uint32_t k = stage_k[slot];
                    const uint32_t dst = gdelta[((k - sub) >> shift) & dmask] + slot;
                    if (kout) kout[dst] = k + key_add;
                    vout[dst] = stage_v[slot];
                    if (ranges_enc) {
                        const uint32_t kp = slot > 0 ? stage_k[slot - 1] : ~k, kn = slot + 1 < nvalid ? stage_k[slot + 1] : ~k;
                        uint32_t* const e = ranges_enc + 2 * (size_t)(key_add + k);
                        const uint32_t at = S.base + dst;
                        if (kp != k) atomicMax(e, ~at);
                        if (kn != k) atomicMax(e + 1, at + 1u);
                    }
                }
            }
            if (EARLY && p + gv < nparts) request(p + gv);
        } else {
#pragma unroll 1
            for (uint32_t k = 0; k < 8; ++k) {
                const uint32_t d = tid * 8u + k;
                uint32_t acc = 0;
#pragma unroll
                for (int wv = 0; wv < FE_WAVES; ++wv) { const uint32_t cw = cnt16[(uint32_t)wv * 2048u + d]; cnt16[(uint32_t)wv * 2048u + d] = (uint16_t)acc; acc += cw; }
                gdelta[d] = dexl[d] + (d < nbins ? hist[(size_t)d * nbtot + row] : 0u);
            }
            __syncthreads();
#pragma unroll
            for (int r = 0; r < ITEMS; ++r) {
                if (vmask & (1u << r)) {
                    uint32_t kk = key[r];
                    asm volatile("" : "+v"(kk));
                    const uint32_t d = ((kk - sub) >> shift) & dmask;
                    const uint32_t dst = gdelta[d] + cnt16[wave * 2048u + d] + rank[r];
                    if (kout) kout[dst] = key[r] + key_add;
                    vout[dst] = val[r];
                }
            }
            if (EARLY && p + gv < nparts) request(p + gv);
        }
    }
}

static inline int fe_items_for(uint64_t n_total) {
    static const uint64_t thr = [] { const char* e = getenv("DVS_FE_ITEMS8_BELOW"); return e ? (uint64_t)atoll(e) : 1500000ull; }();
    return n_total <= thr ? 8 : 16;
}

size_t dvs_fe_hist_words(uint64_t max_elems, int n_views, int max_bins) {
    const uint64_t rows = (max_elems + (uint64_t)FE_BLOCK * 8 - 1) / ((uint64_t)FE_BLOCK * 8) + (uint64_t)n_views + 6;
    return (size_t)(rows * (uint64_t)max_bins);
}

struct FeSortLaunch {
    hipStream_t st;
    int V;
    int items;
    uint32_t grid_per_view;
    uint32_t* hist; uint32_t nbtot; uint32_t* totals;
    int rank_atomic;
};

static hipError_t fe_launch_pass(const FeSortLaunch& L, const uint32_t* kin, const uint32_t* vin, uint32_t* kout, uint32_t* vout, DvsSeg* seg_in,
                                 DvsSeg* seg_out, int adaptive, int pass, int shift, int bits, int cull, uint32_t key_add_per_view,
                                 const uint32_t* kred, uint32_t* ranges_enc = nullptr, int key16 = 0) {
    const dim3 grid(L.grid_per_view * (uint32_t)L.V), blk(FE_BLOCK);
    const int maxbins = adaptive ? FE_MAXBINS : (1 << bits);
    const dim3 rgrid((uint32_t)((maxbins + FE_WAVES - 1) / FE_WAVES) * (uint32_t)L.V);
#define FE_PASS(I, A)                                                                                                                          \
    do {                                                                                                                                       \
        hipLaunchKernelGGL(k_seg_hist<I>, grid, blk, 0, L.st, kin, seg_in, L.V, adaptive, pass, shift, bits, cull, L.hist, L.nbtot, kred, key16); \
        hipLaunchKernelGGL(k_seg_rowscan, rgrid, blk, 0, L.st, L.hist, L.nbtot, (const DvsSeg*)seg_in, L.V, adaptive, bits, (uint32_t)(FE_BLOCK * I), L.totals); \
        hipLaunchKernelGGL((k_seg_scatter<I, A>), grid, blk, 0, L.st, kin, vin, kout, vout, (const DvsSeg*)seg_in, seg_out, L.V, adaptive, pass, shift, bits, \
                           cull, key_add_per_view, (const uint32_t*)L.hist, L.nbtot, (const uint32_t*)L.totals, key16, ranges_enc);               \
    } while (0)
    if (L.items == 8) { if (L.rank_atomic) FE_PASS(8, true); else FE_PASS(8, false); }
    else { if (L.rank_atomic) FE_PASS(16, true); else FE_PASS(16, false); }
#undef FE_PASS
    return hipGetLastError();
}

hipError_t dvs_launch_depth_sort(hipStream_t st, int n, int V, uint32_t* keys0, uint32_t* vals0, uint32_t* keys1, uint32_t* vals1,
                                 DvsSeg* seg_all, DvsSeg* seg_vis, const uint32_t* kred, uint32_t* hist, uint32_t* totals, int rank_atomic) {
    if (n <= 0 || V <= 0) return hipSuccess;
    FeSortLaunch L;
    L.st = st; L.V = V; L.items = fe_items_for((uint64_t)n * V); L.rank_atomic = rank_atomic;
    const uint32_t part = (uint32_t)FE_BLOCK * L.items;
    L.grid_per_view = ((uint32_t)n + part - 1) / part;
    L.hist = hist; L.nbtot = L.grid_per_view * (uint32_t)V + 1; L.totals = totals;
    hipError_t e;
    if ((e = fe_launch_pass(L, keys0, nullptr, keys1, vals1, seg_all, seg_vis, 1, 0, 0, 0, 1, 0, kred)) != hipSuccess) return e;
    if ((e = fe_launch_pass(L, keys1, vals1, keys0, vals0, seg_vis, nullptr, 1, 1, 0, 0, 0, 0, nullptr)) != hipSuccess) return e;
    return fe_launch_pass(L, keys0, vals0, nullptr, vals1, seg_vis, nullptr, 1, 2, 0, 0, 0, 0, nullptr);
}
uint32_t dvs_depth_sort_rows_per_view(int n, int V) {
    const uint32_t part = (uint32_t)FE_BLOCK * fe_items_for((uint64_t)n * V);
    return ((uint32_t)n + part - 1) / part;
}

static void fe_split_bits(int bits, int* npass, int widths[4]) {
    int np = (bits + FE_REORDER_BITS - 1) / FE_REORDER_BITS;
    if (np < 1) np = 1;
    if (np > 4) np = 4;
    int left = bits;
    for (int k = 0; k < np; ++k) { const int wdt = (left + (np - k) - 1) / (np - k); widths[k] = wdt > 0 ? wdt : 1; left -= wdt; }
    *npass = np;
}
uint32_t dvs_fe_part_for(uint64_t grid_elems) { return (uint32_t)FE_BLOCK * (uint32_t)fe_items_for(grid_elems); }

hipError_t dvs_launch_seg_sort(hipStream_t st, int V, uint32_t* keys0, uint32_t* vals0, uint32_t* keys1, uint32_t* vals1, DvsSeg* seg, int bit_lo, int bits,
                               uint64_t grid_elems, uint32_t part, uint32_t nbtot, uint32_t* hist, uint32_t* totals, uint32_t key_add_per_view,
                               int* result_in, uint32_t* ranges_enc, int write_last_keys, int first_keys16, int rank_atomic) {
    if (result_in) *result_in = 0;
    if (V <= 0 || bits <= 0) return hipSuccess;
    int npass, widths[4];
    fe_split_bits(bits, &npass, widths);
    FeSortLaunch L;
    L.st = st; L.V = V; L.items = (int)(part / FE_BLOCK); L.rank_atomic = rank_atomic;
    uint64_t per_view = (grid_elems + (uint64_t)V - 1) / (uint64_t)V;
    uint64_t g = (per_view + part - 1) / part + 1;
    if (g > 65535u * 16u) g = 65535u * 16u;
    L.grid_per_view = (uint32_t)(g < 1 ? 1 : g);
    L.hist = hist; L.nbtot = nbtot; L.totals = totals;
    uint32_t* kk[2] = {keys0, keys1};
    uint32_t* vv[2] = {vals0, vals1};
    int c = 0, shift = bit_lo;
    for (int k = 0; k < npass; ++k) {
        const bool last = k == npass - 1;
        hipError_t e = fe_launch_pass(L, kk[c], vv[c], (last && !write_last_keys) ? nullptr : kk[c ^ 1], vv[c ^ 1], seg, nullptr, 0, k, shift, widths[k], 0,
                                      last ? key_add_per_view : 0u, nullptr, last ? ranges_enc : nullptr, (k == 0 && first_keys16) ? 1 : 0);
        if (e != hipSuccess) return e;
        shift += widths[k];
        c ^= 1;
    }
    if (result_in) *result_in = c;
    return hipSuccess;
}

__global__ void __launch_bounds__(FE_BLOCK)
k_fe_probe_rank_atomic(uint32_t* __restrict__ bad, uint32_t seed) {
    __shared__ uint32_t cnt_a[FE_WAVES * 256];
    __shared__ uint16_t cnt_b[FE_WAVES * 512];
    const uint32_t lane = fe_lane(), wave = threadIdx.x >> 6;
    uint32_t errs = 0;
    for (uint32_t pat = 0; pat < 24; ++pat) {
        for (uint32_t e = threadIdx.x; e < FE_WAVES * 256; e += FE_BLOCK) cnt_a[e] = 0u;
        for (uint32_t e = threadIdx.x; e < FE_WAVES * 512; e += FE_BLOCK) cnt_b[e] = 0;
        __syncthreads();
        const uint32_t bits = pat < 8 ? 9u : 1u + (pat - 8u) % 9u;
        for (uint32_t r = 0; r < 16; ++r) {
            uint32_t h = (lane * 0x9E3779B1u) ^ ((blockIdx.x * FE_WAVES + wave) * 0x85EBCA6Bu) ^ ((pat * 16u + r) * 0xC2B2AE35u) ^ seed;
            h ^= h >> 15; h *= 0x2C1B3C6Du; h ^= h >> 12;
            uint32_t d;
            switch (pat) {
                case 0: d = 5u; break;
                case 1: d = 6u + (lane & 1u); break;
                case 2: d = lane >> 1; break;
                case 3: d = lane / 3u; break;
                case 4: d = lane >> 5; break;
                case 5: d = lane & 7u; break;
                case 6: d = (lane & 1u) ? 511u : (h & 3u); break;
                case 7: d = 63u - lane; break;
                default: d = h & ((1u << bits) - 1u); break;
            }
            const bool valid = (h >> 20 & 15u) != 0u || pat < 8;
            uint32_t ra = 0, rb = 0;
            if (valid) {
                const uint32_t old = atomicAdd(&cnt_a[wave * 256u + (d >> 1)], (d & 1u) ? 0x10000u : 1u);
                ra = (d & 1u) ? (old >> 16) : (old & 0xFFFFu);
            }
            const uint64_t peers = fe_match(d, valid, 9u);
            const uint32_t below = __builtin_amdgcn_mbcnt_hi((uint32_t)(peers >> 32), __builtin_amdgcn_mbcnt_lo((uint32_t)peers, 0u));
            if (valid) {
                const uint32_t prev = cnt_b[wave * 512u + d];
                if (below == 0) cnt_b[wave * 512u + d] = (uint16_t)(prev + (uint32_t)__popcll(peers));
                rb = prev + below;
            }
            errs += (valid && ra != rb) ? 1u : 0u;
        }
        __syncthreads();
    }
    if (errs) atomicAdd(bad, errs);
}
hipError_t dvs_fe_probe_rank_atomic(hipStream_t st, uint32_t* bad_dev ) {
    hipLaunchKernelGGL(k_fe_probe_rank_atomic, dim3(512), dim3(FE_BLOCK), 0, st, bad_dev, 0x1234567u);
    hipLaunchKernelGGL(k_fe_probe_rank_atomic, dim3(512), dim3(FE_BLOCK), 0, st, bad_dev, 0x89ABCDEu);
    return hipGetLastError();
}

template <int FMT> struct FeRect;
template <> struct FeRect<DVS_FE_RECT_U8> {
    typedef uint32_t T;
    static __device__ __forceinline__ uint32_t count(T r) { return ((r >> 16) & 0xFFu) * (r >> 24); }
    static __device__ __forceinline__ uint32_t minx(T r) { return r & 0xFFu; }
    static __device__ __forceinline__ uint32_t miny(T r) { return (r >> 8) & 0xFFu; }
    static __device__ __forceinline__ uint32_t width(T r) { return (r >> 16) & 0xFFu; }
    static __device__ __forceinline__ T zero() { return 0u; }
};
template <> struct FeRect<DVS_FE_RECT_U16> {
    typedef uint2 T;
    static __device__ __forceinline__ uint32_t count(T r) { return ((r.x >> 16) - (r.x & 0xFFFFu)) * ((r.y >> 16) - (r.y & 0xFFFFu)); }
    static __device__ __forceinline__ uint32_t minx(T r) { return r.x & 0xFFFFu; }
    static __device__ __forceinline__ uint32_t miny(T r) { return r.y & 0xFFFFu; }
    static __device__ __forceinline__ uint32_t width(T r) { return (r.x >> 16) - (r.x & 0xFFFFu); }
    static __device__ __forceinline__ T zero() { return make_uint2(0u, 0u); }
};
template <> struct FeRect<DVS_FE_RECT_TIGHT> {
    typedef uint4 T;
    static __device__ __forceinline__ uint32_t count(T r) {
        const uint32_t both = r.z & r.w;
        return both == 0xFFFFFFFFu ? ((r.x >> 16) - (r.x & 0xFFFFu)) * ((r.y >> 16) - (r.y & 0xFFFFu)) : (uint32_t)(__popc(r.z) + __popc(r.w));
    }
    static __device__ __forceinline__ uint32_t minx(T r) { return r.x & 0xFFFFu; }
    static __device__ __forceinline__ uint32_t miny(T r) { return r.y & 0xFFFFu; }
    static __device__ __forceinline__ uint32_t width(T r) { return (r.x >> 16) - (r.x & 0xFFFFu); }
    static __device__ __forceinline__ T zero() { return make_uint4(0u, 0u, 0u, 0u); }
};

template <int FMT>
__global__ void __launch_bounds__(FE_BLOCK)
k_seg_blocksum(int n, int V, uint32_t nbv, uint32_t nsb, const DvsSeg* __restrict__ seg_vis, const uint32_t* __restrict__ sorted_ids,
               const typename FeRect<FMT>::T* __restrict__ rect, typename FeRect<FMT>::T* __restrict__ rect_sorted,
               uint32_t* __restrict__ block_sums, unsigned long long* __restrict__ super) {
    __shared__ uint32_t wsum[4][FE_WAVES];
    const uint32_t view = blockIdx.x % (uint32_t)V, blk0 = (blockIdx.x / (uint32_t)V) * 4u;
    const uint32_t nvis = seg_vis[view].count;
    if (blk0 * FE_BLOCK >= nvis) return;
    const size_t o = (size_t)view * n;
    const uint32_t lane = fe_lane(), wave = threadIdx.x >> 6;
    uint32_t id[4];
#pragma unroll
    for (int k = 0; k < 4; ++k) { const uint32_t j = (blk0 + (uint32_t)k) * FE_BLOCK + threadIdx.x; id[k] = j < nvis ? sorted_ids[o + j] : 0u; }
    typename FeRect<FMT>::T r[4];
#pragma unroll
    for (int k = 0; k < 4; ++k) r[k] = rect[o + id[k]];
#pragma unroll
    for (int k = 0; k < 4; ++k) {
        const uint32_t j = (blk0 + (uint32_t)k) * FE_BLOCK + threadIdx.x;
        uint32_t v = 0;
        if (j < nvis) { rect_sorted[o + j] = r[k]; v = FeRect<FMT>::count(r[k]); }
        const uint32_t s = fe_wave_sum(v);
        if (lane == 0) wsum[k][wave] = s;
    }
    __syncthreads();
    if (threadIdx.x < 4) {
        const uint32_t k = threadIdx.x, blk = blk0 + k;
        uint32_t tot = 0;
#pragma unroll
        for (int wv = 0; wv < FE_WAVES; ++wv) tot += wsum[k][wv];
        if (blk < nbv) block_sums[(size_t)view * nbv + blk] = tot;
        const uint32_t t4 = tot + (uint32_t)__shfl_down(tot, 1, 64) + (uint32_t)__shfl_down(tot, 2, 64) + (uint32_t)__shfl_down(tot, 3, 64);
        if (k == 0 && t4) atomicAdd(&super[((size_t)view * nsb + (blk0 >> 8)) * DVS_FE_SUPER_STRIDE], (unsigned long long)t4);
    }
}

__global__ void __launch_bounds__(1024)
k_seg_totals(int V, uint32_t nsb, const unsigned long long* __restrict__ super, uint32_t* __restrict__ superexcl, DvsSeg* __restrict__ seg_tile,
             uint32_t tile_part, unsigned long long* __restrict__ total, unsigned long long capacity) {
    __shared__ unsigned long long vsum[DVS_MAX_VIEWS];
    const uint32_t lane = fe_lane(), wave = threadIdx.x >> 6;
    if (wave < (uint32_t)V) {
        unsigned long long carry = 0ull;
        for (uint32_t c0 = 0; c0 < nsb; c0 += 64) {
            const uint32_t i = c0 + lane;
            const unsigned long long v = i < nsb ? super[((size_t)wave * nsb + i) * DVS_FE_SUPER_STRIDE] : 0ull;
            unsigned long long inc = v;
#pragma unroll
            for (int k = 1; k < 64; k <<= 1) { const unsigned long long o = __shfl_up(inc, k, 64); if (lane >= (uint32_t)k) inc += o; }
            const unsigned long long ex = carry + inc - v;
            if (i < nsb) superexcl[(size_t)wave * nsb + i] = ex > 0xFFFFFFFFull ? 0xFFFFFFFFu : (uint32_t)ex;
            carry += __shfl(inc, 63, 64);
        }
        if (lane == 0) vsum[wave] = carry;
    }
    __syncthreads();
    if (threadIdx.x == 0) {
        unsigned long long start = 0ull;
        uint32_t prow = 0;
        for (int v = 0; v < V; ++v) {
            const unsigned long long end = start + vsum[v];
            const unsigned long long cs = start < capacity ? start : capacity, ce = end < capacity ? end : capacity;
            DvsSeg s;
            s.base = (uint32_t)cs; s.count = (uint32_t)(ce - cs); s.pstart = prow; s.sub = 0u; s.bits = 0u; s._r0 = s._r1 = s._r2 = 0u;
            seg_tile[v] = s;
            prow += (s.count + tile_part - 1) / tile_part;
            start = end;
        }
        total[0] = start;
        if (start > capacity) total[1] += 1ull;
    }
}

__device__ __forceinline__ uint32_t fe_nth_set_bit64(uint32_t lo, uint32_t hi, uint32_t t) {
    uint32_t w = lo, base = 0;
    const uint32_t c = (uint32_t)__popc(lo);
    if (t >= c) { t -= c; w = hi; base = 32u; }
#pragma unroll
    for (uint32_t h = 16u; h >= 1u; h >>= 1) {
        const uint32_t cl = (uint32_t)__popc(w & ((1u << h) - 1u));
        if (t >= cl) { t -= cl; w >>= h; base += h; }
    }
    return base;
}

__device__ __forceinline__ uint32_t fe_wave_incl_max(uint32_t v) {
#define FE_DPP_MAX(ctrl, rmask) { const uint32_t o_ = (uint32_t)__builtin_amdgcn_update_dpp(0, (int)v, ctrl, rmask, 0xF, false); v = v > o_ ? v : o_; }
    FE_DPP_MAX(0x111, 0xF); FE_DPP_MAX(0x112, 0xF); FE_DPP_MAX(0x114, 0xF); FE_DPP_MAX(0x118, 0xF);
    FE_DPP_MAX(0x142, 0xA);
    FE_DPP_MAX(0x143, 0xC);
#undef FE_DPP_MAX
    return v;
}
template <int FMT>
__global__ void __launch_bounds__(FE_BLOCK)
k_seg_duplicate(int n, int V, uint32_t nbv, uint32_t nsb, const DvsSeg* __restrict__ seg_vis, const DvsSeg* __restrict__ seg_tile,
                const uint32_t* __restrict__ sorted_ids, const typename FeRect<FMT>::T* __restrict__ rect_sorted,
                const uint32_t* __restrict__ block_sums, const uint32_t* __restrict__ superexcl, int tiles_x,
                uint32_t* __restrict__ inst_tile, uint32_t* __restrict__ inst_splat, unsigned long long capacity, int key16 ) {
    __shared__ uint32_t tmp[FE_WAVES];
    __shared__ uint32_t s_pre[FE_BLOCK];
    __shared__ uint32_t s_id[FE_BLOCK];
    __shared__ uint32_t s_tile[FE_BLOCK];
    __shared__ uint32_t s_w[FE_BLOCK];
    __shared__ uint32_t s_mark[FE_BLOCK];
    __shared__ uint2 s_mask[FMT == DVS_FE_RECT_TIGHT ? FE_BLOCK : 1];
    const uint32_t view = blockIdx.x % (uint32_t)V, blk0 = (blockIdx.x / (uint32_t)V) * 2u;
    const uint32_t nvis = seg_vis[view].count;
    if (blk0 * FE_BLOCK >= nvis) return;
    const size_t o = (size_t)view * n;
    const uint32_t lane = fe_lane(), w0 = (threadIdx.x >> 6) * 64u;
    uint32_t id[2] = {0u, 0u};
    typename FeRect<FMT>::T r[2] = {FeRect<FMT>::zero(), FeRect<FMT>::zero()};
#pragma unroll
    for (int h = 0; h < 2; ++h) {
        const uint32_t j = (blk0 + (uint32_t)h) * FE_BLOCK + threadIdx.x;
        if (j < nvis) { id[h] = sorted_ids[o + j]; r[h] = rect_sorted[o + j]; }
    }
    const uint32_t sb = blk0 >> 8, nprev = blk0 & 255u;
    const uint32_t part = threadIdx.x < nprev ? block_sums[(size_t)view * nbv + (size_t)sb * 256 + threadIdx.x] : 0u;
    const unsigned long long vbase = (unsigned long long)seg_tile[view].base + superexcl[(size_t)view * nsb + sb];
    uint32_t before, tot;
    (void)fe_block_excl_scan(part, tmp, &before);
#pragma unroll
    for (int h = 0; h < 2; ++h) {
        if ((blk0 + (uint32_t)h) * FE_BLOCK >= nvis) break;
        const uint32_t touched = FeRect<FMT>::count(r[h]);
        const uint32_t pre = fe_block_excl_scan(touched, tmp, &tot);
        s_pre[threadIdx.x] = pre;
        s_id[threadIdx.x] = (uint32_t)o + id[h];
        s_tile[threadIdx.x] = FeRect<FMT>::miny(r[h]) * (uint32_t)tiles_x + FeRect<FMT>::minx(r[h]);
        s_w[threadIdx.x] = FeRect<FMT>::width(r[h]);
        if constexpr (FMT == DVS_FE_RECT_TIGHT) s_mask[threadIdx.x] = make_uint2(r[h].z, r[h].w);
        const unsigned long long gbase = vbase + before;
        const uint32_t k_beg = (uint32_t)__builtin_amdgcn_readfirstlane((int)pre);
        const uint32_t k_end = (uint32_t)__builtin_amdgcn_readlane((int)(pre + touched), 63);
        uint32_t cur1 = 0;
        for (uint32_t k0 = k_beg; k0 < k_end; k0 += 64u) {
            s_mark[w0 + lane] = 0u;
            __builtin_amdgcn_wave_barrier();
            const uint32_t rel = pre - k0;
            if (touched != 0u && rel < 64u) s_mark[w0 + rel] = lane + 1u;
            __builtin_amdgcn_wave_barrier();
            uint32_t m = s_mark[w0 + lane];
            __builtin_amdgcn_wave_barrier();
            m = fe_wave_incl_max(m);
            m = m > cur1 ? m : cur1;
            cur1 = (uint32_t)__builtin_amdgcn_readlane((int)m, 63);
            const uint32_t k = k0 + lane;
            if (k < k_end) {
                const uint32_t src = w0 + m - 1u, w = s_w[src];
                uint32_t t = k - s_pre[src];
                if constexpr (FMT == DVS_FE_RECT_TIGHT) {
                    const uint2 mk = s_mask[src];
                    if ((mk.x & mk.y) != 0xFFFFFFFFu) t = fe_nth_set_bit64(mk.x, mk.y, t);
                }
                uint32_t q = (uint32_t)((float)t * __builtin_amdgcn_rcpf((float)w));
                int32_t rem = (int32_t)(t - q * w);
                if (rem < 0) { --q; rem += (int32_t)w; } else if (rem >= (int32_t)w) { ++q; rem -= (int32_t)w; }
                const unsigned long long g = gbase + k;
                if (g < capacity) {
                    const uint32_t tile = s_tile[src] + q * (uint32_t)tiles_x + (uint32_t)rem;
                    if (key16) reinterpret_cast<uint16_t*>(inst_tile)[g] = (uint16_t)tile; else inst_tile[g] = tile;
                    inst_splat[g] = s_id[src];
                }
            }
        }
        before += tot;
        __builtin_amdgcn_wave_barrier();
    }
}

hipError_t dvs_launch_seg_binning(hipStream_t st, int n, int V, int rect_fmt, const DvsSeg* seg_vis, DvsSeg* seg_tile, const uint32_t* sorted_ids,
                                  const uint32_t* rect, uint32_t* rect_sorted, uint32_t* block_sums, unsigned long long* super, uint32_t* superexcl,
                                  uint32_t tile_part, unsigned long long* total_dev, unsigned long long capacity, int stage ,
                                  int tiles_x, uint32_t* inst_tile, uint32_t* inst_splat, int key16) {
    if (n <= 0 || V <= 0) return hipSuccess;
    const uint32_t nbv = (uint32_t)((n + FE_BLOCK - 1) / FE_BLOCK), nsb = (nbv + 255u) / 256u;
    const dim3 grid(((nbv + 1u) / 2u) * (uint32_t)V), grid3(((nbv + 3u) / 4u) * (uint32_t)V), blk(FE_BLOCK);
    if (stage == 0) {
#define FE_A3(F) hipLaunchKernelGGL(k_seg_blocksum<F>, grid3, blk, 0, st, n, V, nbv, nsb, seg_vis, sorted_ids, (const FeRect<F>::T*)rect, (FeRect<F>::T*)rect_sorted, block_sums, super)
        if (rect_fmt == DVS_FE_RECT_U8) FE_A3(DVS_FE_RECT_U8); else if (rect_fmt == DVS_FE_RECT_U16) FE_A3(DVS_FE_RECT_U16); else FE_A3(DVS_FE_RECT_TIGHT);
#undef FE_A3
        hipLaunchKernelGGL(k_seg_totals, dim3(1), dim3(1024), 0, st, V, nsb, (const unsigned long long*)super, superexcl, seg_tile, tile_part, total_dev, capacity);
    } else {
#define FE_A4(F) hipLaunchKernelGGL(k_seg_duplicate<F>, grid, blk, 0, st, n, V, nbv, nsb, seg_vis, (const DvsSeg*)seg_tile, sorted_ids, (const FeRect<F>::T*)rect_sorted, \
                                    (const uint32_t*)block_sums, (const uint32_t*)superexcl, tiles_x, inst_tile, inst_splat, capacity, key16)
        if (rect_fmt == DVS_FE_RECT_U8) FE_A4(DVS_FE_RECT_U8); else if (rect_fmt == DVS_FE_RECT_U16) FE_A4(DVS_FE_RECT_U16); else FE_A4(DVS_FE_RECT_TIGHT);
#undef FE_A4
    }
    return hipGetLastError();
}
void dvs_fe_block_counts(int n, uint32_t* nbv, uint32_t* nsb) { *nbv = (uint32_t)((n + FE_BLOCK - 1) / FE_BLOCK); *nsb = (*nbv + 255u) / 256u; }

__global__ void k_seg_init(int n, int V, uint32_t rows_per_view, DvsSeg* __restrict__ seg_all) {
    const int v = threadIdx.x;
    if (v < V) { DvsSeg s; s.base = (uint32_t)v * (uint32_t)n; s.count = (uint32_t)n; s.pstart = (uint32_t)v * rows_per_view; s.sub = 0; s.bits = 8; s._r0 = s._r1 = s._r2 = 0; seg_all[v] = s; }
}
hipError_t dvs_launch_seg_init(hipStream_t st, int n, int V, uint32_t rows_per_view, DvsSeg* seg_all) {
    hipLaunchKernelGGL(k_seg_init, dim3(1), dim3(64), 0, st, n, V, rows_per_view, seg_all);
    return hipGetLastError();
}

__global__ void __launch_bounds__(FE_BLOCK)
k_tile_ranges(uint64_t T_host, const uint64_t* __restrict__ T_dev, const uint32_t* __restrict__ sorted_tile, uint2* __restrict__ ranges) {
    const uint64_t T = T_dev ? (*T_dev < T_host ? *T_dev : T_host) : T_host;
    for (uint64_t q = (uint64_t)blockIdx.x * FE_BLOCK + threadIdx.x; q * 4 < T; q += (uint64_t)gridDim.x * FE_BLOCK) {
        const uint64_t j0 = q * 4;
        uint32_t t[6];
        if (j0 + 4 <= T) {
            const uint4 v = reinterpret_cast<const uint4*>(sorted_tile)[q];
            t[1] = v.x; t[2] = v.y; t[3] = v.z; t[4] = v.w;
        } else {
#pragma unroll
            for (int k = 0; k < 4; ++k) t[1 + k] = j0 + k < T ? sorted_tile[j0 + k] : 0xFFFFFFFFu;
        }
        t[0] = j0 > 0 ? sorted_tile[j0 - 1] : 0xFFFFFFFFu;
        t[5] = j0 + 4 < T ? sorted_tile[j0 + 4] : 0xFFFFFFFFu;
#pragma unroll
        for (int k = 0; k < 4; ++k) {
            const uint64_t j = j0 + k;
            if (j < T) {
                if (j == 0 || t[k] != t[k + 1]) ranges[t[k + 1]].x = (uint32_t)j;
                if (j + 1 == T || t[k + 2] != t[k + 1]) ranges[t[k + 1]].y = (uint32_t)(j + 1);
            }
        }
    }
}

hipError_t dvs_launch_tile_ranges(hipStream_t st, uint64_t T, const uint32_t* sorted_tile, uint32_t* ranges, int tiles, const uint64_t* T_dev,
                                  uint64_t T_expected, bool clear) {
    hipError_t e = clear ? hipMemsetAsync(ranges, 0, (size_t)tiles * 2 * sizeof(uint32_t), st) : hipSuccess;
    if (e != hipSuccess) return e;
    if (T == 0) return hipSuccess;
    const uint64_t T_grid = (T_dev && T_expected > 0 && T_expected < T) ? T_expected : T;
    const uint32_t nb = (uint32_t)((T_grid + 4 * FE_BLOCK - 1) / (4 * FE_BLOCK));
    hipLaunchKernelGGL(k_tile_ranges, dim3(nb), dim3(FE_BLOCK), 0, st, T, T_dev, sorted_tile, (uint2*)ranges);
    return hipGetLastError();
}

__global__ void __launch_bounds__(FE_BLOCK)
k_export_keys(uint64_t T, const uint32_t* __restrict__ sorted_tile, const uint32_t* __restrict__ sorted_splat,
              const float* __restrict__ depth, uint64_t* __restrict__ out) {
    const uint64_t j = (uint64_t)blockIdx.x * FE_BLOCK + threadIdx.x;
    if (j >= T) return;
    out[j] = ((uint64_t)sorted_tile[j] << 32) | (uint64_t)__float_as_uint(depth[sorted_splat[j]]);
}

hipError_t dvs_launch_export_keys(hipStream_t st, uint64_t T, const uint32_t* sorted_tile, const uint32_t* sorted_splat,
                                  const float* depth, uint64_t* out_keys) {
    if (T == 0) return hipSuccess;
    const uint32_t nb = (uint32_t)((T + FE_BLOCK - 1) / FE_BLOCK);
    hipLaunchKernelGGL(k_export_keys, dim3(nb), dim3(FE_BLOCK), 0, st, T, sorted_tile, sorted_splat, depth, out_keys);
    return hipGetLastError();
}
```

### include/dvs_raster.h

```cpp
#ifndef DVS_RASTER_H
#define DVS_RASTER_H

#include <stddef.h>
#include <stdint.h>

#ifdef __cplusplus
extern "C" {
#endif

#define DVS_TILE 16
#define DVS_SH_REST 15

enum {
    DVS_OK = 0,
    DVS_ERR_INVALID = 1,
    DVS_ERR_HIP = 2,
    DVS_ERR_CAPACITY = 3,
    DVS_ERR_STATE = 4,
    DVS_ERR_UNSUPPORTED = 5
};

typedef struct dvs_splats {
    const float* pos;
    const float* sh0;
    const float* shN;
    const float* opacity;
    const float* scale;
    const float* rot;
    int32_t n;
    int32_t _pad;
} dvs_splats;

typedef struct dvs_camera {
    float view[16];
    float proj[16];
    float tan_fovx, tan_fovy;
    float focal_x, focal_y;
    float campos[3];
    int32_t width, height;
    float bg[3];
} dvs_camera;

enum {
    DVS_SHN_ROWS = 0,
    DVS_SHN_TILED = 1
};
#define DVS_SHN_TILE_FLOATS 3072

typedef struct dvs_opts {
    int32_t sh_degree;
    int32_t antialias;
    int32_t absgrad;
    int32_t accumulate;
    int32_t shn_layout;
    int32_t grad_mode;
    int32_t tile_bounds;
    int32_t _reserved[1];
} dvs_opts;

enum { DVS_TILES_CANONICAL = 0, DVS_TILES_TIGHT = 1 };

enum { DVS_GRAD_TRUE = 0, DVS_GRAD_LINEAGE = 1 };

enum { DVS_S2D_X = 0, DVS_S2D_Y = 1, DVS_S2D_CONIC = 2, DVS_S2D_OPACITY = 5, DVS_S2D_RGB = 6, DVS_S2D_DEPTH = 9, DVS_S2D_RADIUS = 10,
       DVS_S2D_CULL = 11, DVS_S2D_FLOATS = 16 };
typedef struct dvs_fwd_state {
    const int32_t*  radii;
    const float*    splat2d;
    const float*    depth;
    const uint32_t* flags;
    const uint32_t* tiles_touched;
    const uint32_t* sorted_tile;
    const uint32_t* sorted_splat;
    const uint32_t* ranges;
    const float*    final_T;
    const uint32_t* n_contrib;
    uint64_t num_rendered;
    int32_t n, width, height, tiles_x, tiles_y, _pad;
} dvs_fwd_state;

typedef struct dvs_splat_grads {
    float* pos;
    float* sh0;
    float* shN;
    float* opacity;
    float* scale;
    float* rot;
    float* absgrad2d;
    float* mean2d;
    float* dcolor;
} dvs_splat_grads;

typedef struct dvs_ctx dvs_ctx;

dvs_ctx* dvs_create(int device, size_t max_splats, int max_w, int max_h);
void     dvs_destroy(dvs_ctx* ctx);

int dvs_raster_forward(dvs_ctx* ctx, void* stream, const dvs_splats* params, const dvs_camera* cam,
                       const dvs_opts* opts, float* out_rgb, dvs_fwd_state* saved, uint64_t* num_rendered);

int dvs_raster_backward(dvs_ctx* ctx, void* stream, const dvs_splats* params, const dvs_camera* cam,
                        const dvs_opts* opts, const float* dL_drgb, const dvs_splat_grads* out);

int dvs_raster_backward_composite(dvs_ctx* ctx, void* stream, const dvs_camera* cam, const dvs_opts* opts, const float* dL_drgb);
int dvs_raster_backward_project(dvs_ctx* ctx, void* stream, const dvs_splats* params, const dvs_camera* cam,
                                const dvs_opts* opts, const dvs_splat_grads* out);

int dvs_raster_backward_project_chunk(dvs_ctx* ctx, void* stream, const dvs_splats* params, const dvs_camera* cam,
                                      const dvs_opts* opts, const dvs_splat_grads* out, int64_t first, int64_t count);

int dvs_raster_backward_dcolor(dvs_ctx* ctx, void* stream, float* dcolor);

int dvs_sh_grad_combine(dvs_ctx* ctx, void* stream, int n, const float* pos, int sh_degree, int n_views, const float* campos,
                        const float* dcolor, float* g_sh0, float* g_shN, int accumulate, int shn_layout);
int dvs_shn_relayout(dvs_ctx* ctx, void* stream, int n, const float* src, float* dst, int to_tiled);

dvs_ctx* dvs_create_views(int device, size_t max_splats, int max_w, int max_h, int max_views);
int dvs_raster_forward_views(dvs_ctx* ctx, void* stream, const dvs_splats* params, const dvs_camera* cams, int n_views,
                             const dvs_opts* opts, float* out_rgb);
int dvs_raster_backward_views(dvs_ctx* ctx, void* stream, const dvs_splats* params, const dvs_camera* cams, int n_views,
                              const dvs_opts* opts, const float* dL_drgb, const dvs_splat_grads* out);

int dvs_raster_forward_views_prepare(dvs_ctx* ctx, void* stream, const dvs_splats* params, const dvs_camera* cams, int n_views,
                                     const dvs_opts* opts, int64_t first, int64_t count);
int dvs_raster_forward_cancel_prepared(dvs_ctx* ctx);
int dvs_get_view_state(dvs_ctx* ctx, int view, dvs_fwd_state* state);

#define DVS_T_UNKNOWN (~0ull)
int dvs_set_async(dvs_ctx* ctx, int enable);
int dvs_get_num_rendered(dvs_ctx* ctx, void* stream, uint64_t* num_rendered);
int dvs_get_arena_info(dvs_ctx* ctx, uint64_t* instance_capacity, uint64_t* grow_events, uint64_t* last_num_rendered, uint64_t* overflows);
int dvs_get_sort_rank_mode(dvs_ctx* ctx);
int dvs_set_export_sorted_tiles(dvs_ctx* ctx, int enable);

int dvs_debug_record_decisions(dvs_ctx* ctx, uint64_t* take_masks, uint64_t capacity_instances);
int dvs_debug_sort_depth_keys(dvs_ctx* ctx, void* stream, const uint32_t* keys, uint64_t n, uint32_t* sorted_ids, uint32_t* n_sorted, uint32_t* digit_bits);

int dvs_set_backward_variant(dvs_ctx* ctx, int variant);
int dvs_set_forward_variant(dvs_ctx* ctx, int variant);
int dvs_set_live_lists(dvs_ctx* ctx, int enable);

int dvs_sort_pairs_u32(dvs_ctx* ctx, void* stream, uint32_t* keys, uint32_t* vals, uint64_t n, int bit_lo, int bit_hi);
int dvs_export_sorted_keys(dvs_ctx* ctx, void* stream, uint64_t* out_keys);

int dvs_get_bwd_intermediates(dvs_ctx* ctx, const float** rows, int* row_floats);
int dvs_keep_bwd_intermediates(dvs_ctx* ctx, int keep);

int dvs_enable_stage_timing(dvs_ctx* ctx, int enable);
int dvs_get_stage_timing(dvs_ctx* ctx, const char*** names, const float** ms);
int dvs_enable_kernel_probe(dvs_ctx* ctx, int enable);
int dvs_read_kernel_probe(dvs_ctx* ctx, float mean_ms[2], int count[2]);

int dvs_memcpy_d2h(dvs_ctx* ctx, void* host_dst, const void* dev_src, size_t bytes);
int dvs_memcpy_h2d(dvs_ctx* ctx, void* dev_dst, const void* host_src, size_t bytes);
void* dvs_device_malloc(dvs_ctx* ctx, size_t bytes);
void  dvs_device_free(dvs_ctx* ctx, void* p);

const char* dvs_last_error(void);
const char* dvs_version(void);

#ifdef __cplusplus
}
#endif
#endif
```

Before: 1839 views/s.

## Replace per-pass radix histogram and rowscan kernels with one-sweep decoupled lookback

Restructures the segmented radix sorts (depth sort and tile sort) to compute all digit histograms in a single upfront kernel. Each scatter pass now resolves its block offsets through decoupled lookback over an epoch-tagged status table, replacing the separate per-pass histogram and rowscan kernels. This removes two kernel launches and a full key read per pass. In exchange it adds spin-waiting on predecessor partitions with a give-up counter, an error path on later forwards, and epoch-parity buffers that are cleared in-kernel. Forward progress depends on partitions being scheduled in order.

```diff
diff --git a/divshot_amd/_lib.py b/divshot_amd/_lib.py
--- a/divshot_amd/_lib.py
+++ b/divshot_amd/_lib.py
@@ -94,6 +94,8 @@
     "dvs_set_async": (C.c_int, [C.c_void_p, C.c_int]),
     "dvs_get_num_rendered": (C.c_int, [C.c_void_p, C.c_void_p, C.POINTER(C.c_uint64)]),
     "dvs_get_sort_rank_mode": (C.c_int, [C.c_void_p]),
+    "dvs_get_sort_giveups": (C.c_int, [C.c_void_p, C.c_void_p, C.POINTER(C.c_uint64)]),
+    "dvs_debug_set_sort_epoch": (C.c_int, [C.c_void_p, C.c_void_p, C.c_uint32]),
     "dvs_debug_sort_depth_keys": (C.c_int, [C.c_void_p, C.c_void_p, C.c_void_p, C.c_uint64, C.c_void_p, C.POINTER(C.c_uint32), C.POINTER(C.c_uint32)]),
     "dvs_set_export_sorted_tiles": (C.c_int, [C.c_void_p, C.c_int]),
     "dvs_get_arena_info": (C.c_int, [C.c_void_p, C.POINTER(C.c_uint64), C.POINTER(C.c_uint64), C.POINTER(C.c_uint64), C.POINTER(C.c_uint64)]),
diff --git a/divshot_amd/csrc/dvs_api.cpp b/divshot_amd/csrc/dvs_api.cpp
--- a/divshot_amd/csrc/dvs_api.cpp
+++ b/divshot_amd/csrc/dvs_api.cpp
@@ -73,7 +73,9 @@
     size_t fe_zero_bytes = 0;
     uint32_t fe_nbv = 0, fe_nsb = 0;
     Buf fe_state;
+    Buf fe_os;
     Buf fe_hist;
+    uint64_t giveup_seen = 0;
     int fe_seg_n = -1, fe_seg_V = -1;
     uint32_t fe_seg_rows = 0;
     Buf g_rows;
@@ -153,16 +155,32 @@
 DvsSeg* fe_seg_vis(dvs_ctx* c) { return c->fe_state.as<DvsSeg>() + DVS_MAX_VIEWS; }
 DvsSeg* fe_seg_tile(dvs_ctx* c) { return c->fe_state.as<DvsSeg>() + 2 * DVS_MAX_VIEWS; }
 uint32_t* fe_superexcl(dvs_ctx* c) { return (uint32_t*)(c->fe_state.as<DvsSeg>() + 3 * DVS_MAX_VIEWS); }
-uint32_t* fe_totals(dvs_ctx* c) { return fe_superexcl(c) + (size_t)c->max_views * c->fe_nsb; }
-uint32_t* fe_block_sums(dvs_ctx* c) { return fe_totals(c) + (size_t)c->max_views * DVS_FE_MAXBINS; }
+uint32_t* fe_block_sums(dvs_ctx* c) { return fe_superexcl(c) + (size_t)c->max_views * c->fe_nsb; }
+uint32_t* fe_os(dvs_ctx* c) { return c->fe_os.as<uint32_t>(); }
+unsigned long long* fe_status(dvs_ctx* c) { return c->fe_hist.as<unsigned long long>(); }
+uint64_t fe_status_words(dvs_ctx* c) { return c->fe_hist.bytes / 8; }
+unsigned long long* fe_giveup(dvs_ctx* c) { return (unsigned long long*)c->total_dev + 2; }
+int ensure_status_table(dvs_ctx* c, size_t words) {
+    const void* old = c->fe_hist.p;
+    int r = c->fe_hist.ensure(words * 8);
+    if (r != DVS_OK || c->fe_hist.p == old) return r;
+    HIPCHECK(hipMemset(c->fe_hist.p, 0, c->fe_hist.bytes));
+    HIPCHECK(hipDeviceSynchronize());
+    return DVS_OK;
+}
 int ensure_frontend_arenas(dvs_ctx* c) {
     dvs_fe_block_counts((int)c->max_splats, &c->fe_nbv, &c->fe_nsb);
     c->fe_zero_bytes = (size_t)DVS_FE_KRED_WORDS * 4 + (size_t)c->max_views * c->fe_nsb * 8 * DVS_FE_SUPER_STRIDE;
     c->fe_zero_bytes = (c->fe_zero_bytes + 255) & ~(size_t)255;
     int r;
-    const size_t state = 3 * DVS_MAX_VIEWS * sizeof(DvsSeg) + ((size_t)c->max_views * c->fe_nsb + (size_t)c->max_views * DVS_FE_MAXBINS + (size_t)c->max_views * c->fe_nbv) * 4;
+    const size_t state = 3 * DVS_MAX_VIEWS * sizeof(DvsSeg) + ((size_t)c->max_views * c->fe_nsb + (size_t)c->max_views * c->fe_nbv) * 4;
     if ((r = c->fe_state.ensure(state)) != DVS_OK) return r;
-    if ((r = c->fe_hist.ensure(dvs_fe_hist_words((uint64_t)c->max_splats * c->max_views, c->max_views, DVS_FE_MAXBINS) * 4)) != DVS_OK) return r;
+    if (!c->fe_os.p) {
+        if ((r = c->fe_os.ensure(dvs_fe_os_words() * 4)) != DVS_OK) return r;
+        HIPCHECK(hipMemset(c->fe_os.p, 0, c->fe_os.bytes));
+        HIPCHECK(hipDeviceSynchronize());
+    }
+    if ((r = ensure_status_table(c, dvs_fe_status_words((uint64_t)c->max_splats * c->max_views, c->max_views, DVS_FE_MAXBINS))) != DVS_OK) return r;
     return DVS_OK;
 }
 
@@ -198,7 +216,7 @@
         if (c->inst_splat[k].bytes / 4 < c->inst_cap) c->inst_cap = c->inst_splat[k].bytes / 4;
     }
     if (c->inst_cap >= (1ull << 32)) c->inst_cap = (1ull << 32) - 1;
-    if ((r = c->fe_hist.ensure(dvs_fe_hist_words(c->inst_cap, c->max_views, 512) * 4)) != DVS_OK) return r;
+    if ((r = ensure_status_table(c, dvs_fe_status_words(c->inst_cap, c->max_views, 512))) != DVS_OK) return r;
     return DVS_OK;
 }
 }
@@ -266,7 +284,7 @@
     (void)hipSetDevice(c->device);
     Buf* all[] = {&c->radii, &c->splat2d, &c->depth, &c->flags, &c->tiles_touched, &c->rect, &c->rect_sorted, &c->key[0], &c->key[1],
                   &c->ids[0], &c->ids[1], &c->inst_tile[0], &c->inst_tile[1], &c->inst_splat[0], &c->inst_splat[1],
-                  &c->tmp_keys, &c->tmp_vals, &c->ranges, &c->final_T, &c->n_contrib, &c->g_rows, &c->dcolor, &c->fe_state, &c->fe_hist, &c->ranges_canon};
+                  &c->tmp_keys, &c->tmp_vals, &c->ranges, &c->final_T, &c->n_contrib, &c->g_rows, &c->dcolor, &c->fe_state, &c->fe_os, &c->fe_hist, &c->ranges_canon};
     for (Buf* b : all) b->release();
     if (c->total_dev) (void)hipFree(c->total_dev);
     if (c->total_host) (void)hipHostFree(c->total_host);
@@ -312,6 +330,12 @@
     StageTimer tm(c, st);
     const int tight = opts->tile_bounds == DVS_TILES_TIGHT ? 1 : 0;
 
+    if (c->total_host[2] != c->giveup_seen) {
+        c->giveup_seen = c->total_host[2];
+        g_last_error = "dvs_raster_forward: a binning sort of an earlier forward on this context gave up waiting for a predecessor partition; "
+                       "that forward's outputs are invalid";
+        return DVS_ERR_SORT_TIMEOUT;
+    }
     uint64_t T = 0, T_expected = 0;
     const uint64_t* T_dev = nullptr;
     int icur = 0;
@@ -352,7 +376,7 @@
                 c->fe_seg_n = n; c->fe_seg_V = V; c->fe_seg_rows = rows;
             }
             HIPCHECK(dvs_launch_depth_sort(st, n, V, c->key[0].as<uint32_t>(), c->ids[0].as<uint32_t>(), c->key[1].as<uint32_t>(), c->ids[1].as<uint32_t>(),
-                                           fe_seg_all(c), fe_seg_vis(c), fe_kred(c), c->fe_hist.as<uint32_t>(), fe_totals(c), c->fe_rank_atomic));
+                                           fe_seg_all(c), fe_seg_vis(c), fe_kred(c), fe_os(c), fe_status(c), fe_status_words(c), fe_giveup(c), c->fe_rank_atomic));
         }
         size_t e2 = tm.mark(); tm.span("depth_sort", e1, e2);
         const uint64_t lastT = c->total_host[0];
@@ -384,11 +408,11 @@
         const bool write_keys = !(fuse_a6 && c->async_T) || c->export_tiles;
         if (n > 0) {
             const uint64_t cap = c->async_T ? c->inst_cap : T;
-            const uint32_t nbtot = (uint32_t)(cap / tile_part) + (uint32_t)V + 2u;
+            (void)cap;
             HIPCHECK(dvs_launch_seg_sort(st, V, c->inst_tile[0].as<uint32_t>(), c->inst_splat[0].as<uint32_t>(), c->inst_tile[1].as<uint32_t>(),
                                          c->inst_splat[1].as<uint32_t>(), fe_seg_tile(c), 0, tiles > 1 ? bits_for((uint32_t)(tiles - 1)) : 1,
-                                         c->async_T ? (T_expected ? T_expected : c->inst_cap) : T, tile_part, nbtot, c->fe_hist.as<uint32_t>(), fe_totals(c),
-                                         (uint32_t)tiles, &icur, fuse_a6 ? ranges_ptr(c) : nullptr, write_keys ? 1 : 0, key16, c->fe_rank_atomic));
+                                         c->async_T ? (T_expected ? T_expected : c->inst_cap) : T, tile_part, fe_os(c), fe_status(c), fe_status_words(c),
+                                         fe_giveup(c), (uint32_t)tiles, &icur, fuse_a6 ? ranges_ptr(c) : nullptr, write_keys ? 1 : 0, key16, c->fe_rank_atomic));
         }
         size_t e6 = tm.mark(); tm.span("tile_sort", e5, e6);
         if (fuse_a6) ranges_encoded = n > 0 ? 1 : 0;
@@ -705,12 +729,12 @@
     int cur = 0;
     {
         if (n > (1ull << 32) - 4097ull) { g_last_error = "dvs_sort_pairs_u32: n must be at most 2^32 - 4097"; return DVS_ERR_CAPACITY; }
-        if ((r = c->fe_hist.ensure(dvs_fe_hist_words(n, 1, 512) * 4)) != DVS_OK) return r;
+        if ((r = ensure_status_table(c, dvs_fe_status_words(n, 1, 512))) != DVS_OK) return r;
         const uint32_t part = dvs_fe_part_for(n);
         HIPCHECK(dvs_launch_seg_init(st, (int)n, 1, 0, fe_seg_all(c)));
         c->fe_seg_n = -1;
-        HIPCHECK(dvs_launch_seg_sort(st, 1, k[0], v[0], k[1], v[1], fe_seg_all(c), bit_lo, bit_hi - bit_lo, n, part, (uint32_t)(n / part) + 3u,
-                                     c->fe_hist.as<uint32_t>(), fe_totals(c), 0u, &cur, nullptr, 1, 0, c->fe_rank_atomic));
+        HIPCHECK(dvs_launch_seg_sort(st, 1, k[0], v[0], k[1], v[1], fe_seg_all(c), bit_lo, bit_hi - bit_lo, n, part, fe_os(c), fe_status(c),
+                                     fe_status_words(c), fe_giveup(c), 0u, &cur, nullptr, 1, 0, c->fe_rank_atomic));
     }
     if (cur == 1) {
         HIPCHECK(hipMemcpyAsync(keys, k[1], n * 4, hipMemcpyDeviceToDevice, st));
@@ -738,7 +762,7 @@
     HIPCHECK(dvs_launch_seg_init(st, (int)n, 1, rows, fe_seg_all(c)));
     c->fe_seg_n = -1;
     HIPCHECK(dvs_launch_depth_sort(st, (int)n, 1, c->key[0].as<uint32_t>(), c->ids[0].as<uint32_t>(), c->key[1].as<uint32_t>(), c->ids[1].as<uint32_t>(),
-                                   fe_seg_all(c), fe_seg_vis(c), fe_kred(c), c->fe_hist.as<uint32_t>(), fe_totals(c), c->fe_rank_atomic));
+                                   fe_seg_all(c), fe_seg_vis(c), fe_kred(c), fe_os(c), fe_status(c), fe_status_words(c), fe_giveup(c), c->fe_rank_atomic));
     DvsSeg sv;
     HIPCHECK(hipMemcpyAsync(&sv, fe_seg_vis(c), sizeof sv, hipMemcpyDeviceToHost, st));
     HIPCHECK(hipStreamSynchronize(st));
@@ -813,6 +837,22 @@
 }
 
 int dvs_get_sort_rank_mode(dvs_ctx* c) { return c ? c->fe_rank_atomic : -1; }
+int dvs_get_sort_giveups(dvs_ctx* c, void* stream, uint64_t* count) {
+    if (!c || !count) { g_last_error = "dvs_get_sort_giveups: null argument"; return DVS_ERR_INVALID; }
+    HIPCHECK(hipSetDevice(c->device));
+    HIPCHECK(hipMemcpyAsync(count, fe_giveup(c), 8, hipMemcpyDeviceToHost, (hipStream_t)stream));
+    HIPCHECK(hipStreamSynchronize((hipStream_t)stream));
+    return DVS_OK;
+}
+int dvs_debug_set_sort_epoch(dvs_ctx* c, void* stream, uint32_t epoch) {
+    if (!c) { g_last_error = "dvs_debug_set_sort_epoch: null context"; return DVS_ERR_INVALID; }
+    HIPCHECK(hipSetDevice(c->device));
+    HIPCHECK(hipMemsetAsync(c->fe_os.p, 0, c->fe_os.bytes, (hipStream_t)stream));
+    HIPCHECK(hipMemsetAsync(c->fe_hist.p, 0, c->fe_hist.bytes, (hipStream_t)stream));
+    HIPCHECK(hipMemcpyAsync(fe_os(c), &epoch, 4, hipMemcpyHostToDevice, (hipStream_t)stream));
+    HIPCHECK(hipStreamSynchronize((hipStream_t)stream));
+    return DVS_OK;
+}
 int dvs_set_export_sorted_tiles(dvs_ctx* c, int enable) {
     if (!c) { g_last_error = "dvs_set_export_sorted_tiles: null context"; return DVS_ERR_INVALID; }
     c->export_tiles = enable != 0;
diff --git a/divshot_amd/csrc/dvs_kernels.h b/divshot_amd/csrc/dvs_kernels.h
--- a/divshot_amd/csrc/dvs_kernels.h
+++ b/divshot_amd/csrc/dvs_kernels.h
@@ -42,17 +42,19 @@
 #define DVS_FE_KRED_WORDS (DVS_MAX_VIEWS * 64 * 16)
 #define DVS_FE_MAXBINS 2048
 #define DVS_FE_SUPER_STRIDE 32
-size_t dvs_fe_hist_words(uint64_t max_elems, int n_views, int max_bins);
+size_t dvs_fe_status_words(uint64_t max_elems, int n_views, int max_bins);
+size_t dvs_fe_os_words();
 uint32_t dvs_depth_sort_rows_per_view(int n, int V);
 uint32_t dvs_fe_part_for(uint64_t grid_elems);
 void dvs_fe_block_counts(int n, uint32_t* nbv, uint32_t* nsb);
 hipError_t dvs_launch_seg_init(hipStream_t st, int n, int V, uint32_t rows_per_view, DvsSeg* seg_all);
 hipError_t dvs_launch_depth_sort(hipStream_t st, int n, int V, uint32_t* keys0, uint32_t* vals0, uint32_t* keys1, uint32_t* vals1,
-                                 DvsSeg* seg_all, DvsSeg* seg_vis, const uint32_t* kred, uint32_t* hist, uint32_t* totals ,
+                                 DvsSeg* seg_all, DvsSeg* seg_vis, const uint32_t* kred, uint32_t* os , unsigned long long* status,
+                                 uint64_t status_words, unsigned long long* giveup ,
                                  int rank_atomic = 0 );
 hipError_t dvs_launch_seg_sort(hipStream_t st, int V, uint32_t* keys0, uint32_t* vals0, uint32_t* keys1, uint32_t* vals1, DvsSeg* seg, int bit_lo, int bits,
-                               uint64_t grid_elems, uint32_t part, uint32_t nbtot, uint32_t* hist, uint32_t* totals, uint32_t key_add_per_view,
-                               int* result_in, uint32_t* ranges_enc = nullptr ,
+                               uint64_t grid_elems, uint32_t part, uint32_t* os, unsigned long long* status, uint64_t status_words,
+                               unsigned long long* giveup, uint32_t key_add_per_view, int* result_in, uint32_t* ranges_enc = nullptr ,
                                int write_last_keys = 1, int first_keys16 = 0 , int rank_atomic = 0);
 hipError_t dvs_fe_probe_rank_atomic(hipStream_t st, uint32_t* bad_dev);
 hipError_t dvs_launch_seg_binning(hipStream_t st, int n, int V, int rect_fmt, const DvsSeg* seg_vis, DvsSeg* seg_tile, const uint32_t* sorted_ids,
diff --git a/divshot_amd/csrc/frontend.hip b/divshot_amd/csrc/frontend.hip
--- a/divshot_amd/csrc/frontend.hip
+++ b/divshot_amd/csrc/frontend.hip
@@ -46,86 +46,147 @@
     return wbase + inc - v;
 }
 
+#define FE_OS_TICKETS 16
+#define FE_OS_TOTALS 256
+#define FE_OS_WORDS (FE_OS_TOTALS + 2 * 4 * DVS_MAX_VIEWS * FE_MAXBINS)
+#define FE_EPOCH_MASK 0x3FFFFFFu
+#define FE_FLAG_AGG 1u
+#define FE_FLAG_INCL 2u
+#define FE_SPIN_LIMIT (1u << 22)
+typedef __attribute__((address_space(1))) unsigned long long fe_gu64;
+
+struct FeDigits { int npass; int shift[4]; int bits[4]; };
+
+__device__ __forceinline__ uint32_t* fe_totals(uint32_t* os, uint32_t par, uint32_t pass, uint32_t view) {
+    return os + FE_OS_TOTALS + ((size_t)(par * 4u + pass) * DVS_MAX_VIEWS + view) * FE_MAXBINS;
+}
+__device__ __forceinline__ uint32_t fe_tag(uint32_t epoch, uint32_t pass, uint32_t flag) { return ((epoch & FE_EPOCH_MASK) << 4) | (pass << 2) | flag; }
+__device__ __forceinline__ void fe_publish(unsigned long long* w, uint32_t tag, uint32_t v) {
+    __hip_atomic_store((fe_gu64*)w, ((unsigned long long)tag << 32) | v, __ATOMIC_RELAXED, __HIP_MEMORY_SCOPE_AGENT);
+}
 
 template <int ITEMS>
 __global__ void __launch_bounds__(FE_BLOCK)
-k_seg_hist(const uint32_t* __restrict__ keys, DvsSeg* __restrict__ seg, int V, int adaptive, int pass, int shift_s, int bits_s, int cull,
-           uint32_t* __restrict__ hist, uint32_t nbtot, const uint32_t* __restrict__ kred, int key16 ) {
-    __shared__ uint32_t h[FE_MAXBINS];
+k_seg_hist(const uint32_t* __restrict__ keys, DvsSeg* __restrict__ seg, int V, int adaptive, FeDigits dg, int cull, const uint32_t* __restrict__ kred,
+           int key16 , uint32_t* __restrict__ os, unsigned long long* __restrict__ status, uint64_t status_words) {
+    __shared__ uint32_t h[3 * FE_MAXBINS];
     constexpr uint32_t PART = FE_BLOCK * ITEMS;
-    const uint32_t lane = fe_lane(), wave = threadIdx.x >> 6, tid = threadIdx.x;
+    const uint32_t lane = fe_lane(), tid = threadIdx.x;
     const uint32_t view = blockIdx.x % (uint32_t)V, w = blockIdx.x / (uint32_t)V, gv = gridDim.x / (uint32_t)V;
-    const uint32_t s_base = seg[view].base, s_count = seg[view].count, s_pstart = seg[view].pstart;
-    uint32_t b = (uint32_t)bits_s, shift = (uint32_t)shift_s, sub = 0u;
+    const uint32_t epoch = os[0] + 1u, par = epoch & 1u;
+    const size_t gtid = (size_t)blockIdx.x * FE_BLOCK + tid, gthreads = (size_t)gridDim.x * FE_BLOCK;
+    for (size_t e = gtid; e < 4 * DVS_MAX_VIEWS; e += gthreads) os[FE_OS_TICKETS + (par ^ 1u) * 4 * DVS_MAX_VIEWS + e] = 0u;
+    for (size_t e = gtid; e < (size_t)4 * DVS_MAX_VIEWS * FE_MAXBINS; e += gthreads) os[FE_OS_TOTALS + (size_t)(par ^ 1u) * 4 * DVS_MAX_VIEWS * FE_MAXBINS + e] = 0u;
+    if ((epoch & FE_EPOCH_MASK) == 0u)
+        for (size_t e = gtid; e < status_words; e += gthreads) status[e] = 0ull;
+    if (blockIdx.x == 0 && tid == 0) os[1] = epoch;
+    const uint32_t s_base = seg[view].base, s_count = seg[view].count;
+    int npass = dg.npass;
+    uint32_t sub = 0u, b0 = 0u;
     if (adaptive) {
-        if (pass == 0) {
-            uint32_t mn = ~kred[((size_t)view * 64 + lane) * 16], mx = kred[((size_t)view * 64 + lane) * 16 + 1];
-#pragma unroll
-            for (int d = 32; d >= 1; d >>= 1) {
-                const uint32_t omn = __shfl_xor(mn, d, 64), omx = __shfl_xor(mx, d, 64);
-                mn = omn < mn ? omn : mn; mx = omx > mx ? omx : mx;
-            }
-            sub = mn; b = 1u;
-            if (mx >= mn) { const uint32_t range = mx - mn; const uint32_t rb = range ? 32u - (uint32_t)__builtin_clz(range) : 0u; b = (rb + 2u) / 3u; if (b < 1u) b = 1u; }
-            else sub = 0u;
-            if (w == 0 && tid == 0) { seg[view].sub = sub; seg[view].bits = b; }
-        } else { sub = seg[view].sub; b = seg[view].bits; }
-        shift = (uint32_t)pass * b;
-    }
-    const uint32_t nbins = 1u << b, dmask = nbins - 1u;
+        uint32_t mn = ~kred[((size_t)view * 64 + lane) * 16], mx = kred[((size_t)view * 64 + lane) * 16 + 1];
+#pragma unroll
+        for (int d = 32; d >= 1; d >>= 1) {
+            const uint32_t omn = __shfl_xor(mn, d, 64), omx = __shfl_xor(mx, d, 64);
+            mn = omn < mn ? omn : mn; mx = omx > mx ? omx : mx;
+        }
+        sub = mn; b0 = 1u;
+        if (mx >= mn) { const uint32_t range = mx - mn; const uint32_t rb = range ? 32u - (uint32_t)__builtin_clz(range) : 0u; b0 = (rb + 2u) / 3u; if (b0 < 1u) b0 = 1u; }
+        else sub = 0u;
+        if (w == 0 && tid == 0) { seg[view].sub = sub; seg[view].bits = b0; }
+        npass = 3;
+    }
+    uint32_t shift[4], dmask[4], hoff[4], hwords = 0;
+#pragma unroll
+    for (int k = 0; k < 4; ++k) {
+        const uint32_t bk = adaptive ? b0 : (uint32_t)dg.bits[k];
+        shift[k] = adaptive ? (uint32_t)k * b0 : (uint32_t)dg.shift[k];
+        dmask[k] = (1u << bk) - 1u;
+        hoff[k] = hwords;
+        if (k < npass) hwords += 1u << bk;
+    }
+    for (uint32_t e = tid; e < hwords; e += FE_BLOCK) h[e] = 0u;
+    __syncthreads();
     const uint32_t nparts = (s_count + PART - 1) / PART;
+    const uint32_t* const kin = keys + s_base;
+    const uint16_t* const kin16 = reinterpret_cast<const uint16_t*>(keys) + s_base;
+    const uint32_t ilast = s_count - 1u;
     for (uint32_t p = w; p < nparts; p += gv) {
-        for (uint32_t e = tid; e < nbins; e += FE_BLOCK) h[e] = 0u;
-        __syncthreads();
-        const uint32_t wb = p * PART + wave * (64 * ITEMS);
+        const uint32_t i0 = p * PART + tid;
         uint32_t kreg[ITEMS];
-        const uint32_t* const kin = keys + s_base;
-        const uint16_t* const kin16 = reinterpret_cast<const uint16_t*>(keys) + s_base;
-        const uint32_t i0 = wb + lane, ilast = s_count - 1u;
         if (key16) {
 #pragma unroll
-            for (int r = 0; r < ITEMS; ++r) { const uint32_t idx = i0 + (uint32_t)r * 64; kreg[r] = kin16[idx < ilast ? idx : ilast]; }
+            for (int r = 0; r < ITEMS; ++r) { const uint32_t idx = i0 + (uint32_t)r * FE_BLOCK; kreg[r] = kin16[idx < ilast ? idx : ilast]; }
         } else {
 #pragma unroll
-            for (int r = 0; r < ITEMS; ++r) { const uint32_t idx = i0 + (uint32_t)r * 64; kreg[r] = kin[idx < ilast ? idx : ilast]; }
+            for (int r = 0; r < ITEMS; ++r) { const uint32_t idx = i0 + (uint32_t)r * FE_BLOCK; kreg[r] = kin[idx < ilast ? idx : ilast]; }
         }
 #pragma unroll
         for (int r = 0; r < ITEMS; ++r) {
-            const bool valid = i0 + (uint32_t)r * 64 <= ilast && !(cull && kreg[r] == FE_CULLED);
-            if (valid) atomicAdd(&h[((kreg[r] - sub) >> shift) & dmask], 1u);
-        }
-        __syncthreads();
-        const size_t row = (size_t)s_pstart + p;
-        for (uint32_t d = tid; d < nbins; d += FE_BLOCK) hist[(size_t)d * nbtot + row] = h[d];
-        __syncthreads();
-    }
-}
-
-__global__ void __launch_bounds__(FE_BLOCK)
-k_seg_rowscan(uint32_t* __restrict__ hist, uint32_t nbtot, const DvsSeg* __restrict__ seg, int V, int adaptive, int bits_s, uint32_t part,
-              uint32_t* __restrict__ totals) {
-    const uint32_t lane = fe_lane(), wave = threadIdx.x >> 6;
-    const uint32_t view = blockIdx.x % (uint32_t)V, d = (blockIdx.x / (uint32_t)V) * FE_WAVES + wave;
-    const uint32_t b = adaptive ? seg[view].bits : (uint32_t)bits_s;
-    if (d >= (1u << b)) return;
-    const uint32_t nparts = (seg[view].count + part - 1) / part;
-    uint32_t* row = hist + (size_t)d * nbtot + seg[view].pstart;
-    uint32_t carry = 0;
-    for (uint32_t c0 = 0; c0 < nparts; c0 += 1024) {
-        uint32_t v[16];
-#pragma unroll
-        for (int k = 0; k < 16; ++k) { const uint32_t i = c0 + (uint32_t)k * 64 + lane; v[k] = i < nparts ? row[i] : 0u; }
-#pragma unroll
-        for (int k = 0; k < 16; ++k) {
-            if (c0 + (uint32_t)k * 64 < nparts) {
-                const uint32_t i = c0 + (uint32_t)k * 64 + lane;
-                const uint32_t inc = fe_wave_incl_scan(v[k]);
-                if (i < nparts) row[i] = carry + inc - v[k];
-                carry += (uint32_t)__builtin_amdgcn_readlane((int)inc, 63);
-            }
-        }
-    }
-    if (lane == 0) totals[(size_t)view * FE_MAXBINS + d] = carry;
+            const bool valid = i0 + (uint32_t)r * FE_BLOCK <= ilast && !(cull && kreg[r] == FE_CULLED);
+            if (valid) {
+                const uint32_t x = kreg[r] - sub;
+#pragma unroll
+                for (int k = 0; k < 4; ++k)
+                    if (k < npass) atomicAdd(&h[hoff[k] + ((x >> shift[k]) & dmask[k])], 1u);
+            }
+        }
+    }
+    __syncthreads();
+#pragma unroll
+    for (int k = 0; k < 4; ++k) {
+        if (k >= npass) break;
+        uint32_t* const tot = fe_totals(os, par, (uint32_t)k, view);
+        for (uint32_t d = tid; d <= dmask[k]; d += FE_BLOCK) { const uint32_t c = h[hoff[k] + d]; if (c) atomicAdd(&tot[d], c); }
+    }
+}
+
+template <int ND, int LB>
+__device__ __forceinline__ void fe_lookback(const unsigned long long* __restrict__ status, uint32_t pstart, uint32_t p, uint32_t sstride, const uint32_t (&d)[ND],
+                                            const bool (&act)[ND], uint32_t tag_agg, uint32_t (&prefix)[ND], unsigned long long* giveup) {
+    int32_t q[ND];
+    bool live[ND];
+#pragma unroll
+    for (int j = 0; j < ND; ++j) { prefix[j] = 0u; q[j] = (int32_t)p - 1; live[j] = act[j] && p > 0u; }
+    const uint32_t tag_incl = tag_agg + (FE_FLAG_INCL - FE_FLAG_AGG);
+    uint32_t spins = 0;
+    for (;;) {
+        bool any_live = false;
+#pragma unroll
+        for (int j = 0; j < ND; ++j) any_live |= live[j];
+        if (!__any(any_live)) break;
+        bool stalled = false;
+#pragma unroll
+        for (int j = 0; j < ND; ++j) {
+            if (!live[j]) continue;
+            unsigned long long wv[LB];
+#pragma unroll
+            for (int k = 0; k < LB; ++k) {
+                const int32_t qq = q[j] - k;
+                wv[k] = qq >= 0 ? __hip_atomic_load((const fe_gu64*)(status + ((size_t)pstart + (uint32_t)qq) * sstride + d[j]), __ATOMIC_RELAXED, __HIP_MEMORY_SCOPE_AGENT) : 0ull;
+            }
+            bool go = true;
+#pragma unroll
+            for (int k = 0; k < LB; ++k) {
+                if (!go || q[j] < 0) break;
+                const uint32_t tg = (uint32_t)(wv[k] >> 32), v = (uint32_t)wv[k];
+                if (tg == tag_incl) { prefix[j] += v; live[j] = false; go = false; }
+                else if (tg == tag_agg) { prefix[j] += v; --q[j]; }
+                else { go = false; stalled = true; }
+            }
+            if (live[j] && q[j] < 0) live[j] = false;
+        }
+        if (__any(stalled)) {
+            if (++spins >= FE_SPIN_LIMIT) {
+                bool any_live = false;
+#pragma unroll
+                for (int j = 0; j < ND; ++j) { any_live |= live[j]; live[j] = false; }
+                if (any_live) atomicAdd(giveup, 1ull);
+                break;
+            }
+            __builtin_amdgcn_s_sleep(1);
+        }
+    }
 }
 
 template <int ITEMS> struct FeScatterLds {
@@ -141,13 +202,14 @@
               uint32_t* __restrict__ keys_out , uint32_t* __restrict__ vals_out,
               const DvsSeg* __restrict__ seg_in, DvsSeg* __restrict__ seg_out ,
               int V, int adaptive, int pass, int shift_s, int bits_s, int cull, uint32_t key_add_per_view,
-              const uint32_t* __restrict__ hist, uint32_t nbtot, const uint32_t* __restrict__ totals,
+              uint32_t* __restrict__ os , unsigned long long* __restrict__ status, uint32_t sstride,
+              unsigned long long* __restrict__ giveup ,
               int key16 ,
               uint32_t* __restrict__ ranges_enc ) {
     constexpr uint32_t PART = FE_BLOCK * ITEMS;
     __shared__ __attribute__((aligned(16))) uint32_t lds[FeScatterLds<ITEMS>::WORDS];
     const uint32_t lane = fe_lane(), wave = threadIdx.x >> 6, tid = threadIdx.x;
-    const uint32_t view = blockIdx.x % (uint32_t)V, w = blockIdx.x / (uint32_t)V, gv = gridDim.x / (uint32_t)V;
+    const uint32_t view = blockIdx.x % (uint32_t)V, w = blockIdx.x / (uint32_t)V;
     const DvsSeg S = seg_in[view];
     const uint32_t b = adaptive ? S.bits : (uint32_t)bits_s;
     const uint32_t shift = adaptive ? (uint32_t)pass * b : (uint32_t)shift_s;
@@ -162,7 +224,11 @@
     uint32_t* const stage_v = stage_k + PART;
     uint32_t* const tmp = lds + (FeScatterLds<ITEMS>::WORDS - 8);
     const uint32_t key_add = key_add_per_view * view;
-    const uint32_t* const vtot = totals + (size_t)view * FE_MAXBINS;
+    const uint32_t epoch = os[1], par = epoch & 1u;
+    if (pass == 0 && blockIdx.x == 0 && tid == 0) os[0] = epoch;
+    const uint32_t* const vtot = fe_totals(os, par, (uint32_t)pass, view);
+    uint32_t* const ticket = os + FE_OS_TICKETS + (par * 4u + (uint32_t)pass) * DVS_MAX_VIEWS + view;
+    const uint32_t tag_agg = fe_tag(epoch, (uint32_t)pass, FE_FLAG_AGG), tag_incl = fe_tag(epoch, (uint32_t)pass, FE_FLAG_INCL);
     const uint32_t* const kin = keys_in + S.base;
     const uint16_t* const kin16 = reinterpret_cast<const uint16_t*>(keys_in) + S.base;
     const uint32_t* const vin = vals_in ? vals_in + S.base : nullptr;
@@ -190,7 +256,10 @@
             for (int r = 0; r < ITEMS; ++r) val[r] = i0 + (uint32_t)r * 64;
         }
     };
-    if (EARLY && w < nparts) request(w);
+    if (tid == 0) tmp[7] = atomicAdd(ticket, 1u);
+    __syncthreads();
+    uint32_t p = tmp[7];
+    if (EARLY && p < nparts) request(p);
 
     uint32_t dex0 = 0, dex1 = 0;
     {
@@ -212,15 +281,11 @@
         }
         if (seg_out && w == 0 && tid == 0) { seg_out[view].base = S.base; seg_out[view].count = tot; seg_out[view].pstart = S.pstart; seg_out[view].sub = S.sub; seg_out[view].bits = S.bits; }
     }
-    for (uint32_t p = w; p < nparts; p += gv) {
-        const size_t row = (size_t)S.pstart + p;
+    while (p < nparts) {
+        unsigned long long* const srow = status + ((size_t)S.pstart + p) * sstride;
+        const uint32_t tag_own = p == 0 ? tag_incl : tag_agg;
         __syncthreads();
         for (uint32_t e = tid; e < cstride * 2u; e += FE_BLOCK) lds[e] = 0u;
-        uint32_t hp0 = 0, hp1 = 0;
-        if (!wide) {
-            if (2u * tid < nbins) hp0 = hist[(size_t)(2u * tid) * nbtot + row];
-            if (2u * tid + 1u < nbins) hp1 = hist[(size_t)(2u * tid + 1u) * nbtot + row];
-        }
         if (!EARLY) request(p);
         __syncthreads();
         const uint32_t i0 = p * PART + wave * (64 * ITEMS) + lane;
@@ -250,6 +315,8 @@
             asm volatile("" : "+v"(rank[r]));
         }
         __syncthreads();
+        uint32_t tk = 0;
+        if (tid == 0) tk = atomicAdd(ticket, 1u);
         if (!wide) {
             uint32_t c0[FE_WAVES], c1[FE_WAVES], bc0 = 0, bc1 = 0;
 #pragma unroll
@@ -257,11 +324,13 @@
                 const uint32_t two = *reinterpret_cast<const uint32_t*>(&cnt16[(uint32_t)wv * 512u + tid * 2u]);
                 c0[wv] = two & 0xFFFFu; c1[wv] = two >> 16; bc0 += c0[wv]; bc1 += c1[wv];
             }
+            const uint32_t d0 = 2u * tid, d1 = 2u * tid + 1u;
+            const bool a0 = d0 < nbins, a1 = d1 < nbins;
+            if (a0) fe_publish(srow + d0, tag_own, bc0);
+            if (a1) fe_publish(srow + d1, tag_own, bc1);
             uint32_t nvalid;
-            uint32_t run = fe_block_excl_scan(bc0 + bc1, tmp, &nvalid);
-            gdelta[tid * 2u] = dex0 + hp0 - run;
-            gdelta[tid * 2u + 1u] = dex1 + hp1 - (run + bc0);
-            uint32_t run1 = run + bc0;
+            const uint32_t run0 = fe_block_excl_scan(bc0 + bc1, tmp, &nvalid);
+            uint32_t run = run0, run1 = run0 + bc0;
 #pragma unroll
             for (int wv = 0; wv < FE_WAVES; ++wv) {
                 *reinterpret_cast<uint32_t*>(&cnt16[(uint32_t)wv * 512u + tid * 2u]) = run | (run1 << 16);
@@ -278,13 +347,28 @@
                     stage_v[pos] = val[r];
                 }
             }
+            {
+                const uint32_t dd[2] = {d0, d1};
+                const bool act[2] = {a0, a1};
+                uint32_t pre[2];
+                fe_lookback<2, 8>(status, S.pstart, p, sstride, dd, act, tag_agg, pre, giveup);
+                if (p > 0) {
+                    if (a0) fe_publish(srow + d0, tag_incl, pre[0] + bc0);
+                    if (a1) fe_publish(srow + d1, tag_incl, pre[1] + bc1);
+                }
+                gdelta[d0] = dex0 + pre[0] - run0;
+                gdelta[d1] = dex1 + pre[1] - (run0 + bc0);
+            }
+            if (tid == 0) tmp[7] = tk;
             __syncthreads();
+            const uint32_t pn = tmp[7];
 #pragma unroll
             for (int i = 0; i < ITEMS; ++i) {
                 const uint32_t slot = (uint32_t)i * FE_BLOCK + tid;
                 if (slot < nvalid) {
                     const uint32_t k = stage_k[slot];
                     const uint32_t dst = gdelta[((k - sub) >> shift) & dmask] + slot;
+                    if (dst > ilast) continue;
                     if (kout) kout[dst] = k + key_add;
                     vout[dst] = stage_v[slot];
                     if (ranges_enc) {
@@ -296,7 +380,8 @@
                     }
                 }
             }
-            if (EARLY && p + gv < nparts) request(p + gv);
+            p = pn;
+            if (EARLY && p < nparts) request(p);
         } else {
 #pragma unroll 1
             for (uint32_t k = 0; k < 8; ++k) {
@@ -304,9 +389,25 @@
                 uint32_t acc = 0;
 #pragma unroll
                 for (int wv = 0; wv < FE_WAVES; ++wv) { const uint32_t cw = cnt16[(uint32_t)wv * 2048u + d]; cnt16[(uint32_t)wv * 2048u + d] = (uint16_t)acc; acc += cw; }
-                gdelta[d] = dexl[d] + (d < nbins ? hist[(size_t)d * nbtot + row] : 0u);
-            }
+                if (d < nbins) fe_publish(srow + d, tag_own, acc);
+                gdelta[d] = acc;
+            }
+#pragma unroll 1
+            for (uint32_t k = 0; k < 8; k += 2) {
+                const uint32_t dd[2] = {tid * 8u + k, tid * 8u + k + 1u};
+                const bool act[2] = {dd[0] < nbins, dd[1] < nbins};
+                uint32_t pre[2];
+                fe_lookback<2, 4>(status, S.pstart, p, sstride, dd, act, tag_agg, pre, giveup);
+#pragma unroll
+                for (int j = 0; j < 2; ++j) {
+                    const uint32_t cnt = gdelta[dd[j]];
+                    if (p > 0 && act[j]) fe_publish(srow + dd[j], tag_incl, pre[j] + cnt);
+                    gdelta[dd[j]] = dexl[dd[j]] + pre[j];
+                }
+            }
+            if (tid == 0) tmp[7] = tk;
             __syncthreads();
+            const uint32_t pn = tmp[7];
 #pragma unroll
             for (int r = 0; r < ITEMS; ++r) {
                 if (vmask & (1u << r)) {
@@ -314,11 +415,13 @@
                     asm volatile("" : "+v"(kk));
                     const uint32_t d = ((kk - sub) >> shift) & dmask;
                     const uint32_t dst = gdelta[d] + cnt16[wave * 2048u + d] + rank[r];
+                    if (dst > ilast) continue;
                     if (kout) kout[dst] = key[r] + key_add;
                     vout[dst] = val[r];
                 }
             }
-            if (EARLY && p + gv < nparts) request(p + gv);
+            p = pn;
+            if (EARLY && p < nparts) request(p);
         }
     }
 }
@@ -328,51 +431,64 @@
     return n_total <= thr ? 8 : 16;
 }
 
-size_t dvs_fe_hist_words(uint64_t max_elems, int n_views, int max_bins) {
+size_t dvs_fe_status_words(uint64_t max_elems, int n_views, int max_bins) {
     const uint64_t rows = (max_elems + (uint64_t)FE_BLOCK * 8 - 1) / ((uint64_t)FE_BLOCK * 8) + (uint64_t)n_views + 6;
     return (size_t)(rows * (uint64_t)max_bins);
 }
+size_t dvs_fe_os_words() { return FE_OS_WORDS; }
 
 struct FeSortLaunch {
     hipStream_t st;
     int V;
     int items;
     uint32_t grid_per_view;
-    uint32_t* hist; uint32_t nbtot; uint32_t* totals;
+    uint32_t* os;
+    unsigned long long* status; uint64_t status_words;
+    unsigned long long* giveup;
     int rank_atomic;
 };
 
-static hipError_t fe_launch_pass(const FeSortLaunch& L, const uint32_t* kin, const uint32_t* vin, uint32_t* kout, uint32_t* vout, DvsSeg* seg_in,
-                                 DvsSeg* seg_out, int adaptive, int pass, int shift, int bits, int cull, uint32_t key_add_per_view,
-                                 const uint32_t* kred, uint32_t* ranges_enc = nullptr, int key16 = 0) {
+static hipError_t fe_launch_hist(const FeSortLaunch& L, const uint32_t* keys, DvsSeg* seg, int adaptive, const FeDigits& dg, int cull,
+                                 const uint32_t* kred, int key16) {
+    uint32_t gv = (L.grid_per_view + 3u) / 4u;
+    const uint32_t fill = (256u + (uint32_t)L.V - 1u) / (uint32_t)L.V;
+    if (gv < fill) gv = fill < L.grid_per_view ? fill : L.grid_per_view;
+    if (gv < 1u) gv = 1u;
+    const dim3 grid(gv * (uint32_t)L.V), blk(FE_BLOCK);
+    if (L.items == 8) hipLaunchKernelGGL(k_seg_hist<8>, grid, blk, 0, L.st, keys, seg, L.V, adaptive, dg, cull, kred, key16, L.os, L.status, L.status_words);
+    else hipLaunchKernelGGL(k_seg_hist<16>, grid, blk, 0, L.st, keys, seg, L.V, adaptive, dg, cull, kred, key16, L.os, L.status, L.status_words);
+    return hipGetLastError();
+}
+
+static hipError_t fe_launch_scatter(const FeSortLaunch& L, const uint32_t* kin, const uint32_t* vin, uint32_t* kout, uint32_t* vout, const DvsSeg* seg_in,
+                                    DvsSeg* seg_out, int adaptive, int pass, int shift, int bits, int cull, uint32_t key_add_per_view,
+                                    uint32_t* ranges_enc = nullptr, int key16 = 0) {
     const dim3 grid(L.grid_per_view * (uint32_t)L.V), blk(FE_BLOCK);
-    const int maxbins = adaptive ? FE_MAXBINS : (1 << bits);
-    const dim3 rgrid((uint32_t)((maxbins + FE_WAVES - 1) / FE_WAVES) * (uint32_t)L.V);
-#define FE_PASS(I, A)                                                                                                                          \
-    do {                                                                                                                                       \
-        hipLaunchKernelGGL(k_seg_hist<I>, grid, blk, 0, L.st, kin, seg_in, L.V, adaptive, pass, shift, bits, cull, L.hist, L.nbtot, kred, key16); \
-        hipLaunchKernelGGL(k_seg_rowscan, rgrid, blk, 0, L.st, L.hist, L.nbtot, (const DvsSeg*)seg_in, L.V, adaptive, bits, (uint32_t)(FE_BLOCK * I), L.totals); \
-        hipLaunchKernelGGL((k_seg_scatter<I, A>), grid, blk, 0, L.st, kin, vin, kout, vout, (const DvsSeg*)seg_in, seg_out, L.V, adaptive, pass, shift, bits, \
-                           cull, key_add_per_view, (const uint32_t*)L.hist, L.nbtot, (const uint32_t*)L.totals, key16, ranges_enc);               \
-    } while (0)
-    if (L.items == 8) { if (L.rank_atomic) FE_PASS(8, true); else FE_PASS(8, false); }
-    else { if (L.rank_atomic) FE_PASS(16, true); else FE_PASS(16, false); }
-#undef FE_PASS
+    const uint32_t sstride = adaptive ? (uint32_t)FE_MAXBINS : 512u;
+#define FE_SCATTER(I, A)                                                                                                                       \
+    hipLaunchKernelGGL((k_seg_scatter<I, A>), grid, blk, 0, L.st, kin, vin, kout, vout, seg_in, seg_out, L.V, adaptive, pass, shift, bits, cull,   \
+                       key_add_per_view, L.os, L.status, sstride, L.giveup, key16, ranges_enc)
+    if (L.items == 8) { if (L.rank_atomic) FE_SCATTER(8, true); else FE_SCATTER(8, false); }
+    else { if (L.rank_atomic) FE_SCATTER(16, true); else FE_SCATTER(16, false); }
+#undef FE_SCATTER
     return hipGetLastError();
 }
 
 hipError_t dvs_launch_depth_sort(hipStream_t st, int n, int V, uint32_t* keys0, uint32_t* vals0, uint32_t* keys1, uint32_t* vals1,
-                                 DvsSeg* seg_all, DvsSeg* seg_vis, const uint32_t* kred, uint32_t* hist, uint32_t* totals, int rank_atomic) {
+                                 DvsSeg* seg_all, DvsSeg* seg_vis, const uint32_t* kred, uint32_t* os, unsigned long long* status, uint64_t status_words,
+                                 unsigned long long* giveup, int rank_atomic) {
     if (n <= 0 || V <= 0) return hipSuccess;
     FeSortLaunch L;
     L.st = st; L.V = V; L.items = fe_items_for((uint64_t)n * V); L.rank_atomic = rank_atomic;
     const uint32_t part = (uint32_t)FE_BLOCK * L.items;
     L.grid_per_view = ((uint32_t)n + part - 1) / part;
-    L.hist = hist; L.nbtot = L.grid_per_view * (uint32_t)V + 1; L.totals = totals;
+    L.os = os; L.status = status; L.status_words = status_words; L.giveup = giveup;
     hipError_t e;
-    if ((e = fe_launch_pass(L, keys0, nullptr, keys1, vals1, seg_all, seg_vis, 1, 0, 0, 0, 1, 0, kred)) != hipSuccess) return e;
-    if ((e = fe_launch_pass(L, keys1, vals1, keys0, vals0, seg_vis, nullptr, 1, 1, 0, 0, 0, 0, nullptr)) != hipSuccess) return e;
-    return fe_launch_pass(L, keys0, vals0, nullptr, vals1, seg_vis, nullptr, 1, 2, 0, 0, 0, 0, nullptr);
+    const FeDigits dg = {3, {0, 0, 0, 0}, {0, 0, 0, 0}};
+    if ((e = fe_launch_hist(L, keys0, seg_all, 1, dg, 1, kred, 0)) != hipSuccess) return e;
+    if ((e = fe_launch_scatter(L, keys0, nullptr, keys1, vals1, seg_all, seg_vis, 1, 0, 0, 0, 1, 0)) != hipSuccess) return e;
+    if ((e = fe_launch_scatter(L, keys1, vals1, keys0, vals0, seg_vis, nullptr, 1, 1, 0, 0, 0, 0)) != hipSuccess) return e;
+    return fe_launch_scatter(L, keys0, vals0, nullptr, vals1, seg_vis, nullptr, 1, 2, 0, 0, 0, 0);
 }
 uint32_t dvs_depth_sort_rows_per_view(int n, int V) {
     const uint32_t part = (uint32_t)FE_BLOCK * fe_items_for((uint64_t)n * V);
@@ -390,8 +506,9 @@
 uint32_t dvs_fe_part_for(uint64_t grid_elems) { return (uint32_t)FE_BLOCK * (uint32_t)fe_items_for(grid_elems); }
 
 hipError_t dvs_launch_seg_sort(hipStream_t st, int V, uint32_t* keys0, uint32_t* vals0, uint32_t* keys1, uint32_t* vals1, DvsSeg* seg, int bit_lo, int bits,
-                               uint64_t grid_elems, uint32_t part, uint32_t nbtot, uint32_t* hist, uint32_t* totals, uint32_t key_add_per_view,
-                               int* result_in, uint32_t* ranges_enc, int write_last_keys, int first_keys16, int rank_atomic) {
+                               uint64_t grid_elems, uint32_t part, uint32_t* os, unsigned long long* status, uint64_t status_words,
+                               unsigned long long* giveup, uint32_t key_add_per_view, int* result_in, uint32_t* ranges_enc, int write_last_keys,
+                               int first_keys16, int rank_atomic) {
     if (result_in) *result_in = 0;
     if (V <= 0 || bits <= 0) return hipSuccess;
     int npass, widths[4];
@@ -402,16 +519,22 @@
     uint64_t g = (per_view + part - 1) / part + 1;
     if (g > 65535u * 16u) g = 65535u * 16u;
     L.grid_per_view = (uint32_t)(g < 1 ? 1 : g);
-    L.hist = hist; L.nbtot = nbtot; L.totals = totals;
+    L.os = os; L.status = status; L.status_words = status_words; L.giveup = giveup;
+    FeDigits dg = {npass, {0, 0, 0, 0}, {1, 1, 1, 1}};
+    {
+        int shift = bit_lo;
+        for (int k = 0; k < npass; ++k) { dg.shift[k] = shift; dg.bits[k] = widths[k]; shift += widths[k]; }
+    }
+    hipError_t e = fe_launch_hist(L, keys0, seg, 0, dg, 0, nullptr, first_keys16);
+    if (e != hipSuccess) return e;
     uint32_t* kk[2] = {keys0, keys1};
     uint32_t* vv[2] = {vals0, vals1};
-    int c = 0, shift = bit_lo;
+    int c = 0;
     for (int k = 0; k < npass; ++k) {
         const bool last = k == npass - 1;
-        hipError_t e = fe_launch_pass(L, kk[c], vv[c], (last && !write_last_keys) ? nullptr : kk[c ^ 1], vv[c ^ 1], seg, nullptr, 0, k, shift, widths[k], 0,
-                                      last ? key_add_per_view : 0u, nullptr, last ? ranges_enc : nullptr, (k == 0 && first_keys16) ? 1 : 0);
+        e = fe_launch_scatter(L, kk[c], vv[c], (last && !write_last_keys) ? nullptr : kk[c ^ 1], vv[c ^ 1], seg, nullptr, 0, k, dg.shift[k], widths[k], 0,
+                              last ? key_add_per_view : 0u, last ? ranges_enc : nullptr, (k == 0 && first_keys16) ? 1 : 0);
         if (e != hipSuccess) return e;
-        shift += widths[k];
         c ^= 1;
     }
     if (result_in) *result_in = c;
diff --git a/include/dvs_raster.h b/include/dvs_raster.h
--- a/include/dvs_raster.h
+++ b/include/dvs_raster.h
@@ -17,7 +17,8 @@
     DVS_ERR_HIP = 2,
     DVS_ERR_CAPACITY = 3,
     DVS_ERR_STATE = 4,
-    DVS_ERR_UNSUPPORTED = 5
+    DVS_ERR_UNSUPPORTED = 5,
+    DVS_ERR_SORT_TIMEOUT = 6
 };
 
 typedef struct dvs_splats {
@@ -131,6 +132,8 @@
 int dvs_get_num_rendered(dvs_ctx* ctx, void* stream, uint64_t* num_rendered);
 int dvs_get_arena_info(dvs_ctx* ctx, uint64_t* instance_capacity, uint64_t* grow_events, uint64_t* last_num_rendered, uint64_t* overflows);
 int dvs_get_sort_rank_mode(dvs_ctx* ctx);
+int dvs_get_sort_giveups(dvs_ctx* ctx, void* stream, uint64_t* count);
+int dvs_debug_set_sort_epoch(dvs_ctx* ctx, void* stream, uint32_t epoch);
 int dvs_set_export_sorted_tiles(dvs_ctx* ctx, int enable);
 
 int dvs_debug_record_decisions(dvs_ctx* ctx, uint64_t* take_masks, uint64_t capacity_instances);
```

After: 1673 views/s, median of 2. -9.0%, worse.
